# NilFoundation/vote-saver-protocol

Hardware: AMD Instinct MI355X
Metric: G1 MSM points/sec at 2^20 (Groth16 prover hot path) (higher is better)
Workload: dtype u32; 1 GPU; 2^20-point BLS12-381 G1 Pippenger MSM per GPU, PLAIN bases k_i*G (no table of window multiples; the library's 28-bit-limb copy keeps phi(P) = (beta x, y) beside every P for the endomorphism split), uniform scalars, bases and scalars resident in HBM; N ranks = one 2^20*N-point MSM sharded by contiguous chunk, RCCL all-gather of Jacobian partial sums + fold; points_per_gpu=1048576, window_bits=16, windows=8, endomorphism_split=True, msms_in_flight=4, bases_precomputed_window_multiples=False, bases_memory_bytes_per_point=352

## Files before the change

vote_saver_protocol_amd/csrc/fp28.h:

```cpp
#pragma once
#include "curve.h"

namespace vsp {

struct Fp28 {
    uint32_t l[14];
    VSP_HD static Fp28 zero() { Fp28 r; for (int i = 0; i < 14; i++) r.l[i] = 0; return r; }
};
VSP_HD bool is_zero(const Fp28 &a) { uint32_t o = 0; for (int i = 0; i < 14; i++) o |= a.l[i]; return o == 0; }
struct alignas(128) Affine28 { Fp28 x, y; };
static_assert(sizeof(Fp28) == 56 && sizeof(Affine28) == 128, "G1 table rows are one 128-byte line");
struct XYZZ28 { Fp28 X, Y, ZZ, ZZZ; };
struct Fp2x28 { Fp28 c0, c1; VSP_HD static Fp2x28 zero() { Fp2x28 r; r.c0 = Fp28::zero(); r.c1 = Fp28::zero(); return r; } };
struct Fp28L { Fp28 v; VSP_HD static Fp28L zero() { Fp28L r; r.v = Fp28::zero(); return r; } };
VSP_HD bool is_zero(const Fp2x28 &a) { return is_zero(a.c0) && is_zero(a.c1); }
struct alignas(256) Affine28x2 { Fp28 xc0, xc1, yc0, yc1; };
static_assert(sizeof(Affine28x2) == 256, "G2 table rows are two 128-byte lines");

#if defined(__HIP_DEVICE_COMPILE__)
__device__ __forceinline__ Fp28 fp28_zero() { Fp28 r; for (int i = 0; i < 14; i++) r.l[i] = 0; return r; }
__device__ __forceinline__ Fp28 fp28_const(const uint32_t (&c)[14]) { Fp28 r; for (int i = 0; i < 14; i++) r.l[i] = c[i]; return r; }
__device__ __forceinline__ bool fp28_all_zero(const Fp28 &a) { uint32_t o = 0; for (int i = 0; i < 14; i++) o |= a.l[i]; return o == 0; }
__device__ __forceinline__ bool fp28_equals(const Fp28 &a, const uint32_t (&c)[14]) { uint32_t o = 0; for (int i = 0; i < 14; i++) o |= a.l[i] ^ c[i]; return o == 0; }

#if defined(VSP_PORTABLE_MUL)
__device__ __noinline__ void mont28_portable(uint32_t *r, const uint32_t *a, const uint32_t *b, const uint32_t *c, const uint32_t *d) {
    uint32_t m[14];
    uint64_t acc = 0;
    for (int k = 0; k < 27; k++) {
        for (int i = (k > 13 ? k - 13 : 0); i <= (k < 13 ? k : 13); i++) {
            acc += (uint64_t)a[i] * b[k - i];
            if (c) acc += (uint64_t)c[i] * d[k - i];
        }
        if (k < 14) {
            for (int i = 0; i < k; i++) acc += (uint64_t)m[i] * FP28_P[k - i];
            m[k] = ((uint32_t)acc * 0xffcfffdu) & 0x0FFFFFFFu;
            acc += (uint64_t)m[k] * FP28_P[0];
        } else {
            for (int i = k - 13; i < 14; i++) acc += (uint64_t)m[i] * FP28_P[k - i];
            r[k - 14] = (uint32_t)acc & 0x0FFFFFFFu;
        }
        acc >>= 28;
    }
    r[13] = (uint32_t)acc;
}
__device__ __forceinline__ Fp28 mul28(const Fp28 &a, const Fp28 &b) { Fp28 r; mont28_portable(r.l, a.l, b.l, nullptr, nullptr); return r; }
__device__ __forceinline__ Fp28 sqr28(const Fp28 &a) { Fp28 r; mont28_portable(r.l, a.l, a.l, nullptr, nullptr); return r; }
__device__ __forceinline__ Fp28 mul28x2(const Fp28 &a, const Fp28 &b, const Fp28 &c, const Fp28 &d) { Fp28 r; mont28_portable(r.l, a.l, b.l, c.l, d.l); return r; }
#else
__device__ __forceinline__ Fp28 mul28(const Fp28 &a, const Fp28 &b) {
    Fp28 r;
    __builtin_amdgcn_sched_barrier(0);
    mont_mul28_asm(r.l, a.l, b.l);
    __builtin_amdgcn_sched_barrier(0);
    (void)&mont_mul28_holder<0>;
    return r;
}
__device__ __forceinline__ Fp28 sqr28(const Fp28 &a) {
    Fp28 r, a2;
#pragma unroll
    for (int i = 0; i < 14; i++) a2.l[i] = 2u * a.l[i];
    __builtin_amdgcn_sched_barrier(0);
    mont_sqr28_asm(r.l, a.l, a2.l);
    __builtin_amdgcn_sched_barrier(0);
    (void)&mont_sqr28_holder<0>;
    return r;
}
__device__ __forceinline__ Fp28 mul28x2(const Fp28 &a, const Fp28 &b, const Fp28 &c, const Fp28 &d) {
    Fp28 r;
    __builtin_amdgcn_sched_barrier(0);
    mont_mul28x2_asm(r.l, a.l, b.l, c.l, d.l);
    __builtin_amdgcn_sched_barrier(0);
    (void)&mont_mul28x2_holder<0>;
    return r;
}
#endif
__device__ __forceinline__ Fp28 sub28(const Fp28 &a, const uint32_t (&K)[14], const Fp28 &b) {
    Fp28 r;
#pragma unroll
    for (int i = 0; i < 14; i++) r.l[i] = a.l[i] + K[i] - b.l[i];
    return r;
}
__device__ __forceinline__ Fp28 neg28(const uint32_t (&K)[14], const Fp28 &b) {
    Fp28 r;
#pragma unroll
    for (int i = 0; i < 14; i++) r.l[i] = K[i] - b.l[i];
    return r;
}
__device__ __forceinline__ Fp28 norm28(const Fp28 &a) {
    Fp28 r;
    uint32_t c = 0;
#pragma unroll
    for (int i = 0; i < 13; i++) { uint32_t t = a.l[i] + c; r.l[i] = t & 0x0FFFFFFFu; c = t >> 28; }
    r.l[13] = a.l[13] + c;
    return r;
}
__device__ __forceinline__ bool fp28_product_is_zero(const Fp28 &a) { return fp28_all_zero(a) || fp28_equals(a, FP28_P); }

__device__ __forceinline__ Fp28 fp_to_fp28(const Fp &m) {
    __builtin_amdgcn_sched_barrier(0);
    Fp c = from_mont(m);
    __builtin_amdgcn_sched_barrier(0);
    Fp28 s;
#pragma unroll
    for (int i = 0; i < 14; i++) {
        const int bit = 28 * i, w = bit >> 5, sh = bit & 31;
        uint64_t v = c.l[w];
        if (w + 1 < 12) v |= (uint64_t)c.l[w + 1] << 32;
        s.l[i] = (uint32_t)(v >> sh) & (i < 13 ? 0x0FFFFFFFu : 0xFFFFFFFFu);
    }
    return mul28(s, fp28_const(FP28_R2));
}
__device__ __forceinline__ Fp fp28_to_fp(const Fp28 &x) {
    Fp28 one = fp28_zero(); one.l[0] = 1;
    Fp28 v = mul28(x, one);
    Fp28 d; uint32_t borrow = 0;
#pragma unroll
    for (int i = 0; i < 14; i++) {
        uint32_t t = v.l[i] - FP28_P[i] - borrow;
        borrow = (i < 13) ? ((t >> 28) & 1u) : (t >> 31);
        d.l[i] = (i < 13) ? (t & 0x0FFFFFFFu) : t;
    }
    if (!borrow) v = d;
    Fp c;
#pragma unroll
    for (int w = 0; w < 12; w++) {
        uint32_t acc = 0;
#pragma unroll
        for (int i = 0; i < 14; i++) {
            const int lo = 28 * i - 32 * w;
            if (lo > -28 && lo < 32) acc |= lo >= 0 ? (v.l[i] << lo) : (v.l[i] >> (-lo));
        }
        c.l[w] = acc;
    }
    __builtin_amdgcn_sched_barrier(0);
    Fp out = to_mont(c);
    __builtin_amdgcn_sched_barrier(0);
    return out;
}

__device__ __forceinline__ bool is_inf28(const Affine28 &p) { return fp28_all_zero(p.x) && fp28_all_zero(p.y); }
__device__ __forceinline__ bool is_inf28(const XYZZ28 &p) { return fp28_all_zero(p.ZZ); }
__device__ __forceinline__ XYZZ28 xyzz28_inf() { XYZZ28 r; r.X = r.Y = r.ZZ = r.ZZZ = fp28_zero(); return r; }
__device__ __forceinline__ XYZZ<Fp> xyzz28_to_fp(const XYZZ28 &a) {
    XYZZ<Fp> r;
    if (is_inf28(a)) return XYZZ<Fp>::inf();
    r.X = fp28_to_fp(a.X); r.Y = fp28_to_fp(a.Y); r.ZZ = fp28_to_fp(a.ZZ); r.ZZZ = fp28_to_fp(a.ZZZ);
    return r;
}

__device__ __forceinline__ bool madd28(XYZZ28 &acc, const Affine28 &q, bool negate) {
    if (is_inf28(q)) return true;
    Fp28 qy = negate ? neg28(FP28_K8_L1, q.y) : q.y;
    if (is_inf28(acc)) { acc.X = q.x; acc.Y = negate ? norm28(qy) : qy; acc.ZZ = fp28_const(FP28_ONE); acc.ZZZ = acc.ZZ; return true; }
    Fp28 U2 = mul28(q.x, acc.ZZ);
    Fp28 S2 = mul28(qy, acc.ZZZ);
    Fp28 P = norm28(sub28(U2, FP28_K32_L1, acc.X));
    Fp28 PP = sqr28(P);
    if (fp28_product_is_zero(PP)) return false;
    Fp28 R = norm28(sub28(S2, FP28_K32_L1, acc.Y));
    Fp28 PPP = mul28(P, PP);
    Fp28 Q = mul28(acc.X, PP);
    Fp28 s;
#pragma unroll
    for (int i = 0; i < 14; i++) s.l[i] = PPP.l[i] + 2u * Q.l[i];
    Fp28 X3 = norm28(sub28(sqr28(R), FP28_K8_L4, s));
    acc.Y = mul28x2(R, sub28(Q, FP28_K32_L1, X3), neg28(FP28_K32_L1, acc.Y), PPP);
    acc.X = X3;
    acc.ZZ = mul28(acc.ZZ, PP);
    acc.ZZZ = mul28(acc.ZZZ, PPP);
    return true;
}
__device__ __forceinline__ XYZZ<Fp28> xyzz28_from_fp(const XYZZ<Fp> &a) {
    XYZZ<Fp28> r;
    if (is_inf(a)) return XYZZ<Fp28>::inf();
    r.X = fp_to_fp28(a.X); r.Y = fp_to_fp28(a.Y); r.ZZ = fp_to_fp28(a.ZZ); r.ZZZ = fp_to_fp28(a.ZZZ);
    return r;
}
__device__ __forceinline__ XYZZ<Fp> xyzz28_to_fp(const XYZZ<Fp28> &a) {
    XYZZ<Fp> r;
    if (fp28_all_zero(a.ZZ)) return XYZZ<Fp>::inf();
    r.X = fp28_to_fp(a.X); r.Y = fp28_to_fp(a.Y); r.ZZ = fp28_to_fp(a.ZZ); r.ZZZ = fp28_to_fp(a.ZZZ);
    return r;
}
__device__ __forceinline__ XYZZ<Fp28> xyzz_dbl28(const XYZZ<Fp28> &a) {
    XYZZ<Fp28> r;
    Fp28 U;
#pragma unroll
    for (int i = 0; i < 14; i++) U.l[i] = 2u * a.Y.l[i];
    Fp28 V = mul28(U, U);
    Fp28 W = mul28(U, V);
    Fp28 S = mul28(a.X, V);
    Fp28 M = sqr28(a.X);
#pragma unroll
    for (int i = 0; i < 14; i++) M.l[i] *= 3u;
    M = norm28(M);
    Fp28 S2;
#pragma unroll
    for (int i = 0; i < 14; i++) S2.l[i] = 2u * S.l[i];
    r.X = norm28(sub28(sqr28(M), FP28_K8_L4, S2));
    r.Y = mul28x2(M, sub28(S, FP28_K32_L1, r.X), neg28(FP28_K32_L1, a.Y), W);
    r.ZZ = mul28(V, a.ZZ);
    r.ZZZ = mul28(W, a.ZZZ);
    return r;
}
__device__ __forceinline__ void xyzz_add(XYZZ<Fp28> &acc, const XYZZ<Fp28> &q) {
    if (fp28_all_zero(q.ZZ)) return;
    if (fp28_all_zero(acc.ZZ)) { acc = q; return; }
    Fp28 U1 = mul28(acc.X, q.ZZ), U2 = mul28(q.X, acc.ZZ);
    Fp28 S1 = mul28(acc.Y, q.ZZZ), S2 = mul28(q.Y, acc.ZZZ);
    Fp28 P = norm28(sub28(U2, FP28_K8_L1, U1));
    Fp28 PP = sqr28(P);
    Fp28 R = norm28(sub28(S2, FP28_K8_L1, S1));
    if (fp28_product_is_zero(PP)) {
        if (fp28_product_is_zero(sqr28(R))) acc = xyzz_dbl28(q); else acc = XYZZ<Fp28>::inf();
        return;
    }
    Fp28 PPP = mul28(P, PP);
    Fp28 Q = mul28(U1, PP);
    Fp28 s;
#pragma unroll
    for (int i = 0; i < 14; i++) s.l[i] = PPP.l[i] + 2u * Q.l[i];
    Fp28 X3 = norm28(sub28(sqr28(R), FP28_K8_L4, s));
    acc.Y = mul28x2(R, sub28(Q, FP28_K32_L1, X3), neg28(FP28_K8_L1, S1), PPP);
    acc.X = X3;
    acc.ZZ = mul28(mul28(acc.ZZ, q.ZZ), PP);
    acc.ZZZ = mul28(mul28(acc.ZZZ, q.ZZZ), PPP);
}


__device__ __forceinline__ Fp28 partner28(const Fp28 &a) {
    Fp28 r;
#pragma unroll
    for (int i = 0; i < 14; i++) r.l[i] = (uint32_t)__builtin_amdgcn_update_dpp(0, (int)a.l[i], 0xB1, 0xF, 0xF, false);
    return r;
}
__device__ __forceinline__ Fp28 select28(bool c, const Fp28 &a, const Fp28 &b) {
    Fp28 r;
#pragma unroll
    for (int i = 0; i < 14; i++) r.l[i] = c ? a.l[i] : b.l[i];
    return r;
}
__device__ __forceinline__ Fp28 mulF2(const Fp28 &a, const Fp28 &b, const uint32_t (&KB)[14]) {
    const bool hi = (threadIdx.x & 1) != 0;
    Fp28 ap = partner28(a), bp = partner28(b);
    Fp28 s1 = select28(hi, bp, b);
    Fp28 s2 = select28(hi, b, neg28(KB, bp));
    return mul28x2(a, s1, ap, s2);
}
__device__ __forceinline__ Fp28 sqrF2(const Fp28 &a, const uint32_t (&KA)[14]) {
    const bool hi = (threadIdx.x & 1) != 0;
    Fp28 ap = partner28(a), sum, dbl;
#pragma unroll
    for (int i = 0; i < 14; i++) { sum.l[i] = a.l[i] + ap.l[i]; dbl.l[i] = 2u * a.l[i]; }
    Fp28 x = select28(hi, ap, sum);
    Fp28 y = select28(hi, dbl, sub28(a, KA, ap));
    return mul28(x, y);
}
__device__ __forceinline__ bool fp28_small_is_zero(const Fp28 &a) {
    return fp28_all_zero(a) || fp28_equals(a, FP28_P) || fp28_equals(a, FP28_2P) || fp28_equals(a, FP28_3P);
}
__device__ __forceinline__ bool pair_all28(bool c) {
    int f = c ? 1 : 0;
    return (f & __builtin_amdgcn_update_dpp(0, f, 0xB1, 0xF, 0xF, false)) != 0;
}
struct AffineHalf28 { Fp28 x, y; };
struct XYZZHalf28 { Fp28 X, Y, ZZ, ZZZ; };
__device__ __forceinline__ XYZZHalf28 xyzz_half28_inf() { XYZZHalf28 r; r.X = r.Y = r.ZZ = r.ZZZ = fp28_zero(); return r; }

__device__ __forceinline__ bool madd28_g2(XYZZHalf28 &acc, const AffineHalf28 &q, bool negate) {
    const bool hi = (threadIdx.x & 1) != 0;
    if (pair_all28(fp28_all_zero(q.x) && fp28_all_zero(q.y))) return true;
    Fp28 qy = negate ? neg28(FP28_K8_L1, q.y) : q.y;
    if (pair_all28(fp28_all_zero(acc.ZZ))) {
        acc.X = q.x; acc.Y = qy;
        acc.ZZ = hi ? fp28_zero() : fp28_const(FP28_ONE); acc.ZZZ = acc.ZZ;
        return true;
    }
    Fp28 U2 = mulF2(q.x, acc.ZZ, FP28_K8_L1);
    Fp28 S2 = mulF2(qy, acc.ZZZ, FP28_K8_L1);
    Fp28 P = norm28(sub28(U2, FP28_K32_L1, acc.X));
    Fp28 PP = sqrF2(P, FP28_K64_L1);
    if (pair_all28(fp28_small_is_zero(PP))) return false;
    Fp28 R = norm28(sub28(S2, FP28_K32_L4, acc.Y));
    Fp28 PPP = mulF2(P, PP, FP28_K8_L1);
    Fp28 Q = mulF2(acc.X, PP, FP28_K8_L1);
    Fp28 s;
#pragma unroll
    for (int i = 0; i < 14; i++) s.l[i] = PPP.l[i] + 2u * Q.l[i];
    Fp28 X3 = norm28(sub28(sqrF2(R, FP28_K64_L1), FP28_K8_L4, s));
    Fp28 D = sub28(Q, FP28_K32_L1, X3);
    Fp28 t1 = mulF2(R, D, FP28_K64_L4);
    Fp28 t2 = mulF2(acc.Y, PPP, FP28_K8_L1);
    acc.Y = sub28(t1, FP28_K8_L1, t2);
    acc.X = X3;
    acc.ZZ = mulF2(acc.ZZ, PP, FP28_K8_L1);
    acc.ZZZ = mulF2(acc.ZZZ, PPP, FP28_K8_L1);
    return true;
}

__device__ __forceinline__ bool is_zero(const Fp28L &a) { return pair_all28(fp28_all_zero(a.v)); }
__device__ __forceinline__ XYZZ<Fp28L> xyzz_dbl28_g2(const XYZZ<Fp28L> &a) {
    XYZZ<Fp28L> r;
    Fp28 Yn = norm28(a.Y.v), U;
#pragma unroll
    for (int i = 0; i < 14; i++) U.l[i] = 2u * Yn.l[i];
    U = norm28(U);
    Fp28 V = sqrF2(U, FP28_K32_L1);
    Fp28 W = mulF2(U, V, FP28_K8_L1);
    Fp28 S = mulF2(a.X.v, V, FP28_K8_L1);
    Fp28 M = sqrF2(a.X.v, FP28_K32_L1);
#pragma unroll
    for (int i = 0; i < 14; i++) M.l[i] *= 3u;
    M = norm28(M);
    Fp28 S2;
#pragma unroll
    for (int i = 0; i < 14; i++) S2.l[i] = 2u * S.l[i];
    Fp28 X3 = norm28(sub28(sqrF2(M, FP28_K8_L1), FP28_K8_L4, S2));
    Fp28 D = sub28(S, FP28_K32_L1, X3);
    Fp28 t1 = mulF2(M, D, FP28_K64_L4);
    Fp28 t2 = mulF2(Yn, W, FP28_K8_L1);
    r.X.v = X3;
    r.Y.v = sub28(t1, FP28_K8_L1, t2);
    r.ZZ.v = mulF2(V, a.ZZ.v, FP28_K8_L1);
    r.ZZZ.v = mulF2(W, a.ZZZ.v, FP28_K8_L1);
    return r;
}
__device__ __forceinline__ void xyzz_add(XYZZ<Fp28L> &acc, const XYZZ<Fp28L> &q) {
    if (pair_all28(fp28_all_zero(q.ZZ.v))) return;
    if (pair_all28(fp28_all_zero(acc.ZZ.v))) { acc = q; return; }
    Fp28 U1 = mulF2(acc.X.v, q.ZZ.v, FP28_K8_L1), U2 = mulF2(q.X.v, acc.ZZ.v, FP28_K8_L1);
    Fp28 S1 = mulF2(acc.Y.v, q.ZZZ.v, FP28_K8_L1), S2 = mulF2(q.Y.v, acc.ZZZ.v, FP28_K8_L1);
    Fp28 P = norm28(sub28(U2, FP28_K8_L1, U1));
    Fp28 PP = sqrF2(P, FP28_K32_L1);
    Fp28 R = norm28(sub28(S2, FP28_K8_L1, S1));
    if (pair_all28(fp28_product_is_zero(PP))) {
        if (pair_all28(fp28_product_is_zero(sqrF2(R, FP28_K32_L1)))) acc = xyzz_dbl28_g2(q); else acc = XYZZ<Fp28L>::inf();
        return;
    }
    Fp28 PPP = mulF2(P, PP, FP28_K8_L1);
    Fp28 Q = mulF2(U1, PP, FP28_K8_L1);
    Fp28 s;
#pragma unroll
    for (int i = 0; i < 14; i++) s.l[i] = PPP.l[i] + 2u * Q.l[i];
    Fp28 X3 = norm28(sub28(sqrF2(R, FP28_K32_L1), FP28_K8_L4, s));
    Fp28 D = sub28(Q, FP28_K32_L1, X3);
    Fp28 t1 = mulF2(R, D, FP28_K64_L4);
    Fp28 t2 = mulF2(S1, PPP, FP28_K8_L1);
    acc.Y.v = sub28(t1, FP28_K8_L1, t2);
    acc.X.v = X3;
    acc.ZZ.v = mulF2(mulF2(acc.ZZ.v, q.ZZ.v, FP28_K8_L1), PP, FP28_K8_L1);
    acc.ZZZ.v = mulF2(mulF2(acc.ZZZ.v, q.ZZZ.v, FP28_K8_L1), PPP, FP28_K8_L1);
}
#else
__device__ __forceinline__ void xyzz_add(XYZZ<Fp28> &, const XYZZ<Fp28> &) {}
__device__ __forceinline__ void xyzz_add(XYZZ<Fp28L> &, const XYZZ<Fp28L> &) {}
#endif

}
```

vote_saver_protocol_amd/csrc/mont_asm_gfx950.h:

```cpp
#pragma once
#include <stdint.h>

namespace vsp {

template <class P> __device__ __attribute__((noinline, used)) void mont_mul_holder_12() {
    static_assert(P::N == 12, "limb count");
    asm volatile(
        "s_branch .Lvsp_mm_12_end\n\t"
        ".p2align 8\n\t"
        "vsp_mm_12:\n\t"
        "s_mov_b32 s0, %[p0]\n\t"
        "s_mov_b32 s1, %[p1]\n\t"
        "s_mov_b32 s2, %[p2]\n\t"
        "s_mov_b32 s3, %[p3]\n\t"
        "s_mov_b32 s4, %[p4]\n\t"
        "s_mov_b32 s5, %[p5]\n\t"
        "s_mov_b32 s6, %[p6]\n\t"
        "s_mov_b32 s7, %[p7]\n\t"
        "s_mov_b32 s8, %[p8]\n\t"
        "s_mov_b32 s9, %[p9]\n\t"
        "s_mov_b32 s10, %[p10]\n\t"
        "s_mov_b32 s11, %[p11]\n\t"
        "s_mov_b32 s12, %[inv]\n\t"
        "v_mov_b32 v36, 0\n\t"
// ... 955 lines not shown
        "v_addc_co_u32 v27, vcc, 0, v27, vcc\n\t"
        "v_mad_u64_u32 v[24:25], vcc, v22, s6, v[24:25]\n\t"
        "v_addc_co_u32 v27, vcc, 0, v27, vcc\n\t"
        "v_mad_u64_u32 v[24:25], vcc, v7, v13, v[24:25]\n\t"
        "v_addc_co_u32 v27, vcc, 0, v27, vcc\n\t"
        "v_mad_u64_u32 v[24:25], vcc, v23, s5, v[24:25]\n\t"
        "v_addc_co_u32 v27, vcc, 0, v27, vcc\n\t"
        "v_mov_b32 v20, v24\n\t"
        "v_mov_b32 v26, v25\n\t"
        "v_mad_u64_u32 v[26:27], vcc, v6, v15, v[26:27]\n\t"
        "v_addc_co_u32_e64 v25, vcc, 0, 0, vcc\n\t"
        "v_mad_u64_u32 v[26:27], vcc, v22, s7, v[26:27]\n\t"
        "v_addc_co_u32 v25, vcc, 0, v25, vcc\n\t"
        "v_mad_u64_u32 v[26:27], vcc, v7, v14, v[26:27]\n\t"
        "v_addc_co_u32 v25, vcc, 0, v25, vcc\n\t"
        "v_mad_u64_u32 v[26:27], vcc, v23, s6, v[26:27]\n\t"
        "v_addc_co_u32 v25, vcc, 0, v25, vcc\n\t"
        "v_mov_b32 v21, v26\n\t"
        "v_mov_b32 v24, v27\n\t"
        "v_mad_u64_u32 v[24:25], vcc, v7, v15, v[24:25]\n\t"
        "v_addc_co_u32_e64 v27, vcc, 0, 0, vcc\n\t"
        "v_mad_u64_u32 v[24:25], vcc, v23, s7, v[24:25]\n\t"
        "v_addc_co_u32 v27, vcc, 0, v27, vcc\n\t"
        "v_mov_b32 v22, v24\n\t"
        "v_mov_b32 v26, v25\n\t"
        "v_mov_b32 v23, v26\n\t"
        "v_subrev_co_u32 v0, vcc, s0, v16\n\t"
        "v_mov_b32 v9, s1\n\t"
        "v_subb_co_u32 v1, vcc, v17, v9, vcc\n\t"
        "v_mov_b32 v10, s2\n\t"
        "v_subb_co_u32 v2, vcc, v18, v10, vcc\n\t"
        "v_mov_b32 v11, s3\n\t"
        "v_subb_co_u32 v3, vcc, v19, v11, vcc\n\t"
        "v_mov_b32 v12, s4\n\t"
        "v_subb_co_u32 v4, vcc, v20, v12, vcc\n\t"
        "v_mov_b32 v13, s5\n\t"
        "v_subb_co_u32 v5, vcc, v21, v13, vcc\n\t"
        "v_mov_b32 v14, s6\n\t"
        "v_subb_co_u32 v6, vcc, v22, v14, vcc\n\t"
        "v_mov_b32 v15, s7\n\t"
        "v_subb_co_u32 v7, vcc, v23, v15, vcc\n\t"
        "v_cndmask_b32 v16, v0, v16, vcc\n\t"
        "v_cndmask_b32 v17, v1, v17, vcc\n\t"
        "v_cndmask_b32 v18, v2, v18, vcc\n\t"
        "v_cndmask_b32 v19, v3, v19, vcc\n\t"
        "v_cndmask_b32 v20, v4, v20, vcc\n\t"
        "v_cndmask_b32 v21, v5, v21, vcc\n\t"
        "v_cndmask_b32 v22, v6, v22, vcc\n\t"
        "v_cndmask_b32 v23, v7, v23, vcc\n\t"
        "s_nop 4\n\t"
        "s_setpc_b64 s[30:31]\n\t"
        ".Lvsp_mm_8_end:\n\t"
        :
        : [p0] "i"(P::MOD[0]), [p1] "i"(P::MOD[1]), [p2] "i"(P::MOD[2]), [p3] "i"(P::MOD[3]), [p4] "i"(P::MOD[4]), [p5] "i"(P::MOD[5]), [p6] "i"(P::MOD[6]), [p7] "i"(P::MOD[7]), [inv] "i"(P::INV)
        : "vcc", "scc", "s30", "s31", "s0", "s1", "s2", "s3", "s4", "s5", "s6", "s7", "s8", "s9", "s10", "s11", "s12", "v0", "v1", "v2", "v3", "v4", "v5", "v6", "v7", "v8", "v9", "v10", "v11", "v12", "v13", "v14", "v15", "v16", "v17", "v18", "v19", "v20", "v21", "v22", "v23", "v24", "v25", "v26", "v27");
}

template <class P> __device__ __forceinline__ void mont_mul_asm_8(uint32_t *r, uint32_t *a, uint32_t *b) {
    asm("s_getpc_b64 s[30:31]\n\t"
        "s_add_u32 s30, s30, vsp_mm_8@rel32@lo+4\n\t"
        "s_addc_u32 s31, s31, vsp_mm_8@rel32@hi+12\n\t"
        "s_swappc_b64 s[30:31], s[30:31]"
        : "={v16}"(r[0]), "={v17}"(r[1]), "={v18}"(r[2]), "={v19}"(r[3]), "={v20}"(r[4]), "={v21}"(r[5]), "={v22}"(r[6]), "={v23}"(r[7]), "+{v0}"(a[0]), "+{v1}"(a[1]), "+{v2}"(a[2]), "+{v3}"(a[3]), "+{v4}"(a[4]), "+{v5}"(a[5]), "+{v6}"(a[6]), "+{v7}"(a[7]), "+{v8}"(b[0]), "+{v9}"(b[1]), "+{v10}"(b[2]), "+{v11}"(b[3]), "+{v12}"(b[4]), "+{v13}"(b[5]), "+{v14}"(b[6]), "+{v15}"(b[7])
        :
        : "vcc", "scc", "s30", "s31", "s0", "s1", "s2", "s3", "s4", "s5", "s6", "s7", "s8", "s9", "s10", "s11", "s12", "v24", "v25", "v26", "v27");
}

static constexpr uint32_t FP28_P[14] = {0xfffaaabu, 0xfefffffu, 0x3ffffb9u, 0xfffeb15u, 0x6241eabu, 0xa0f6b0fu, 0xf6730d2u, 0xf38512bu, 0x4774b84u, 0x4bacd76u, 0xba7b643u, 0xe69a4b1u, 0x1ea397fu, 0x1a011u};
static constexpr uint32_t FP28_ONE[14] = {0x347fcb8u, 0xd800000u, 0x2b119u, 0xcde6d2u, 0xc7212e0u, 0x83a2090u, 0x37669fu, 0xda0f73eu, 0x9b09b42u, 0x1297bb0u, 0x515d98fu, 0x12ca7cu, 0x659fcfau, 0x577au};
static constexpr uint32_t FP28_R2[14] = {0x10370edu, 0x6d1c345u, 0xe243d62u, 0xec45c53u, 0x3b1d65au, 0x93317du, 0xb4f36a0u, 0x5d74088u, 0xc10ea72u, 0x865d118u, 0x7320a75u, 0xfd5cd50u, 0xcc8a759u, 0xc8d4u};
static constexpr uint32_t FP28_K8_L1[14] = {0x1ffd5558u, 0x1f7ffffeu, 0x1ffffdceu, 0x1fff58a8u, 0x1120f55eu, 0x107b587au, 0x1b398694u, 0x19c2895eu, 0x13ba5c26u, 0x15d66bb1u, 0x1d3db219u, 0x134d258cu, 0x1f51cbfeu, 0xd0087u};
static constexpr uint32_t FP28_K8_L4[14] = {0x4ffd5558u, 0x4f7ffffbu, 0x4ffffdcbu, 0x4fff58a5u, 0x4120f55bu, 0x407b5877u, 0x4b398691u, 0x49c2895bu, 0x43ba5c23u, 0x45d66baeu, 0x4d3db216u, 0x434d2589u, 0x4f51cbfbu, 0xd0084u};
static constexpr uint32_t FP28_K32_L1[14] = {0x1ff55560u, 0x1dfffffeu, 0x1ffff73eu, 0x1ffd62a6u, 0x1483d57eu, 0x11ed61ebu, 0x1ce61a53u, 0x170a257du, 0x1ee9709du, 0x1759aec7u, 0x14f6c868u, 0x1d349636u, 0x1d472ffbu, 0x340222u};
static constexpr uint32_t FP28_K32_L4[14] = {0x4ff55560u, 0x4dfffffbu, 0x4ffff73bu, 0x4ffd62a3u, 0x4483d57bu, 0x41ed61e8u, 0x4ce61a50u, 0x470a257au, 0x4ee9709au, 0x4759aec4u, 0x44f6c865u, 0x4d349633u, 0x4d472ff8u, 0x34021fu};
static constexpr uint32_t FP28_K64_L1[14] = {0x1feaaac0u, 0x1bfffffeu, 0x1fffee7eu, 0x1ffac54eu, 0x1907aafeu, 0x13dac3d7u, 0x19cc34a7u, 0x1e144afcu, 0x1dd2e13bu, 0x1eb35d90u, 0x19ed90d1u, 0x1a692c6du, 0x1a8e5ff8u, 0x680446u};
static constexpr uint32_t FP28_K64_L4[14] = {0x4feaaac0u, 0x4bfffffbu, 0x4fffee7bu, 0x4ffac54bu, 0x4907aafbu, 0x43dac3d4u, 0x49cc34a4u, 0x4e144af9u, 0x4dd2e138u, 0x4eb35d8du, 0x49ed90ceu, 0x4a692c6au, 0x4a8e5ff5u, 0x680443u};
static constexpr uint32_t FP28_2P[14] = {0xfff5556u, 0xfdfffffu, 0x7ffff73u, 0xfffd62au, 0xc483d57u, 0x41ed61eu, 0xece61a5u, 0xe70a257u, 0x8ee9709u, 0x9759aecu, 0x74f6c86u, 0xcd34963u, 0x3d472ffu, 0x34022u};
static constexpr uint32_t FP28_3P[14] = {0xfff0001u, 0xfcfffffu, 0xbffff2du, 0xfffc13fu, 0x26c5c03u, 0xe2e412eu, 0xe359277u, 0xda8f383u, 0xd65e28eu, 0xe306862u, 0x2f722c9u, 0xb3cee15u, 0x5beac7fu, 0x4e033u};
template <int Instance> __device__ __attribute__((noinline, used)) void mont_mul28_holder() {
    asm volatile(
        "s_branch .Lvsp_mm28_end\n\t"
        ".p2align 8\n\t"
        "vsp_mm28:\n\t"
        "s_mov_b32 s0, 0xfffaaab\n\t"
        "s_mov_b32 s1, 0xfefffff\n\t"
        "s_mov_b32 s2, 0x3ffffb9\n\t"
        "s_mov_b32 s3, 0xfffeb15\n\t"
        "s_mov_b32 s4, 0x6241eab\n\t"
        "s_mov_b32 s5, 0xa0f6b0f\n\t"
        "s_mov_b32 s6, 0xf6730d2\n\t"
        "s_mov_b32 s7, 0xf38512b\n\t"
        "s_mov_b32 s8, 0x4774b84\n\t"
        "s_mov_b32 s9, 0x4bacd76\n\t"
        "s_mov_b32 s10, 0xba7b643\n\t"
        "s_mov_b32 s11, 0xe69a4b1\n\t"
        "s_mov_b32 s12, 0x1ea397f\n\t"
        "s_mov_b32 s13, 0x1a011\n\t"
        "s_mov_b32 s14, 0xffcfffd\n\t"
        "s_mov_b32 s15, 0xfffffff\n\t"
        "v_mov_b32 v42, 0\n\t"
        "v_mov_b32 v43, 0\n\t"
        "v_mad_u64_u32 v[42:43], vcc, v0, v14, v[42:43]\n\t"
        "v_mul_lo_u32 v44, v42, s14\n\t"
        "v_and_b32 v28, s15, v44\n\t"
        "v_mad_u64_u32 v[42:43], vcc, v28, s0, v[42:43]\n\t"
        "v_lshrrev_b64 v[42:43], 28, v[42:43]\n\t"
        "v_mad_u64_u32 v[42:43], vcc, v0, v15, v[42:43]\n\t"
        "v_mad_u64_u32 v[42:43], vcc, v1, v14, v[42:43]\n\t"
        "v_mad_u64_u32 v[42:43], vcc, v28, s1, v[42:43]\n\t"
        "v_mul_lo_u32 v44, v42, s14\n\t"
        "v_and_b32 v29, s15, v44\n\t"
        "v_mad_u64_u32 v[42:43], vcc, v29, s0, v[42:43]\n\t"
        "v_lshrrev_b64 v[42:43], 28, v[42:43]\n\t"
        "v_mad_u64_u32 v[42:43], vcc, v0, v16, v[42:43]\n\t"
        "v_mad_u64_u32 v[42:43], vcc, v1, v15, v[42:43]\n\t"
        "v_mad_u64_u32 v[42:43], vcc, v2, v14, v[42:43]\n\t"
        "v_mad_u64_u32 v[42:43], vcc, v28, s2, v[42:43]\n\t"
        "v_mad_u64_u32 v[42:43], vcc, v29, s1, v[42:43]\n\t"
        "v_mul_lo_u32 v44, v42, s14\n\t"
        "v_and_b32 v30, s15, v44\n\t"
        "v_mad_u64_u32 v[42:43], vcc, v30, s0, v[42:43]\n\t"
        "v_lshrrev_b64 v[42:43], 28, v[42:43]\n\t"
        "v_mad_u64_u32 v[42:43], vcc, v0, v17, v[42:43]\n\t"
        "v_mad_u64_u32 v[42:43], vcc, v1, v16, v[42:43]\n\t"
        "v_mad_u64_u32 v[42:43], vcc, v2, v15, v[42:43]\n\t"
        "v_mad_u64_u32 v[42:43], vcc, v3, v14, v[42:43]\n\t"
        "v_mad_u64_u32 v[42:43], vcc, v28, s3, v[42:43]\n\t"
        "v_mad_u64_u32 v[42:43], vcc, v29, s2, v[42:43]\n\t"
        "v_mad_u64_u32 v[42:43], vcc, v30, s1, v[42:43]\n\t"
        "v_mul_lo_u32 v44, v42, s14\n\t"
        "v_and_b32 v31, s15, v44\n\t"
        "v_mad_u64_u32 v[42:43], vcc, v31, s0, v[42:43]\n\t"
        "v_lshrrev_b64 v[42:43], 28, v[42:43]\n\t"
        "v_mad_u64_u32 v[42:43], vcc, v0, v18, v[42:43]\n\t"
        "v_mad_u64_u32 v[42:43], vcc, v1, v17, v[42:43]\n\t"
        "v_mad_u64_u32 v[42:43], vcc, v2, v16, v[42:43]\n\t"
        "v_mad_u64_u32 v[42:43], vcc, v3, v15, v[42:43]\n\t"
        "v_mad_u64_u32 v[42:43], vcc, v4, v14, v[42:43]\n\t"
        "v_mad_u64_u32 v[42:43], vcc, v28, s4, v[42:43]\n\t"
        "v_mad_u64_u32 v[42:43], vcc, v29, s3, v[42:43]\n\t"
        "v_mad_u64_u32 v[42:43], vcc, v30, s2, v[42:43]\n\t"
        "v_mad_u64_u32 v[42:43], vcc, v31, s1, v[42:43]\n\t"
        "v_mul_lo_u32 v44, v42, s14\n\t"
        "v_and_b32 v32, s15, v44\n\t"
        "v_mad_u64_u32 v[42:43], vcc, v32, s0, v[42:43]\n\t"
        "v_lshrrev_b64 v[42:43], 28, v[42:43]\n\t"
        "v_mad_u64_u32 v[42:43], vcc, v0, v19, v[42:43]\n\t"
        "v_mad_u64_u32 v[42:43], vcc, v1, v18, v[42:43]\n\t"
        "v_mad_u64_u32 v[42:43], vcc, v2, v17, v[42:43]\n\t"
        "v_mad_u64_u32 v[42:43], vcc, v3, v16, v[42:43]\n\t"
        "v_mad_u64_u32 v[42:43], vcc, v4, v15, v[42:43]\n\t"
        "v_mad_u64_u32 v[42:43], vcc, v5, v14, v[42:43]\n\t"
        "v_mad_u64_u32 v[42:43], vcc, v28, s5, v[42:43]\n\t"
        "v_mad_u64_u32 v[42:43], vcc, v29, s4, v[42:43]\n\t"
        "v_mad_u64_u32 v[42:43], vcc, v30, s3, v[42:43]\n\t"
        "v_mad_u64_u32 v[42:43], vcc, v31, s2, v[42:43]\n\t"
        "v_mad_u64_u32 v[42:43], vcc, v32, s1, v[42:43]\n\t"
        "v_mul_lo_u32 v44, v42, s14\n\t"
        "v_and_b32 v33, s15, v44\n\t"
        "v_mad_u64_u32 v[42:43], vcc, v33, s0, v[42:43]\n\t"
        "v_lshrrev_b64 v[42:43], 28, v[42:43]\n\t"
        "v_mad_u64_u32 v[42:43], vcc, v0, v20, v[42:43]\n\t"
        "v_mad_u64_u32 v[42:43], vcc, v1, v19, v[42:43]\n\t"
        "v_mad_u64_u32 v[42:43], vcc, v2, v18, v[42:43]\n\t"
        "v_mad_u64_u32 v[42:43], vcc, v3, v17, v[42:43]\n\t"
        "v_mad_u64_u32 v[42:43], vcc, v4, v16, v[42:43]\n\t"
// ... 329 lines not shown
        "v_mad_u64_u32 v[42:43], vcc, v11, v23, v[42:43]\n\t"
        "v_mad_u64_u32 v[42:43], vcc, v12, v22, v[42:43]\n\t"
        "v_mad_u64_u32 v[42:43], vcc, v13, v21, v[42:43]\n\t"
        "v_mad_u64_u32 v[42:43], vcc, v35, s13, v[42:43]\n\t"
        "v_mad_u64_u32 v[42:43], vcc, v36, s12, v[42:43]\n\t"
        "v_mad_u64_u32 v[42:43], vcc, v37, s11, v[42:43]\n\t"
        "v_mad_u64_u32 v[42:43], vcc, v38, s10, v[42:43]\n\t"
        "v_mad_u64_u32 v[42:43], vcc, v39, s9, v[42:43]\n\t"
        "v_mad_u64_u32 v[42:43], vcc, v40, s8, v[42:43]\n\t"
        "v_mad_u64_u32 v[42:43], vcc, v41, s7, v[42:43]\n\t"
        "v_and_b32 v34, s15, v42\n\t"
        "v_lshrrev_b64 v[42:43], 28, v[42:43]\n\t"
        "v_mad_u64_u32 v[42:43], vcc, v8, v27, v[42:43]\n\t"
        "v_mad_u64_u32 v[42:43], vcc, v9, v26, v[42:43]\n\t"
        "v_mad_u64_u32 v[42:43], vcc, v10, v25, v[42:43]\n\t"
        "v_mad_u64_u32 v[42:43], vcc, v11, v24, v[42:43]\n\t"
        "v_mad_u64_u32 v[42:43], vcc, v12, v23, v[42:43]\n\t"
        "v_mad_u64_u32 v[42:43], vcc, v13, v22, v[42:43]\n\t"
        "v_mad_u64_u32 v[42:43], vcc, v36, s13, v[42:43]\n\t"
        "v_mad_u64_u32 v[42:43], vcc, v37, s12, v[42:43]\n\t"
        "v_mad_u64_u32 v[42:43], vcc, v38, s11, v[42:43]\n\t"
        "v_mad_u64_u32 v[42:43], vcc, v39, s10, v[42:43]\n\t"
        "v_mad_u64_u32 v[42:43], vcc, v40, s9, v[42:43]\n\t"
        "v_mad_u64_u32 v[42:43], vcc, v41, s8, v[42:43]\n\t"
        "v_and_b32 v35, s15, v42\n\t"
        "v_lshrrev_b64 v[42:43], 28, v[42:43]\n\t"
        "v_mad_u64_u32 v[42:43], vcc, v9, v27, v[42:43]\n\t"
        "v_mad_u64_u32 v[42:43], vcc, v10, v26, v[42:43]\n\t"
        "v_mad_u64_u32 v[42:43], vcc, v11, v25, v[42:43]\n\t"
        "v_mad_u64_u32 v[42:43], vcc, v12, v24, v[42:43]\n\t"
        "v_mad_u64_u32 v[42:43], vcc, v13, v23, v[42:43]\n\t"
        "v_mad_u64_u32 v[42:43], vcc, v37, s13, v[42:43]\n\t"
        "v_mad_u64_u32 v[42:43], vcc, v38, s12, v[42:43]\n\t"
        "v_mad_u64_u32 v[42:43], vcc, v39, s11, v[42:43]\n\t"
        "v_mad_u64_u32 v[42:43], vcc, v40, s10, v[42:43]\n\t"
        "v_mad_u64_u32 v[42:43], vcc, v41, s9, v[42:43]\n\t"
        "v_and_b32 v36, s15, v42\n\t"
        "v_lshrrev_b64 v[42:43], 28, v[42:43]\n\t"
        "v_mad_u64_u32 v[42:43], vcc, v10, v27, v[42:43]\n\t"
        "v_mad_u64_u32 v[42:43], vcc, v11, v26, v[42:43]\n\t"
        "v_mad_u64_u32 v[42:43], vcc, v12, v25, v[42:43]\n\t"
        "v_mad_u64_u32 v[42:43], vcc, v13, v24, v[42:43]\n\t"
        "v_mad_u64_u32 v[42:43], vcc, v38, s13, v[42:43]\n\t"
        "v_mad_u64_u32 v[42:43], vcc, v39, s12, v[42:43]\n\t"
        "v_mad_u64_u32 v[42:43], vcc, v40, s11, v[42:43]\n\t"
        "v_mad_u64_u32 v[42:43], vcc, v41, s10, v[42:43]\n\t"
        "v_and_b32 v37, s15, v42\n\t"
        "v_lshrrev_b64 v[42:43], 28, v[42:43]\n\t"
        "v_mad_u64_u32 v[42:43], vcc, v11, v27, v[42:43]\n\t"
        "v_mad_u64_u32 v[42:43], vcc, v12, v26, v[42:43]\n\t"
        "v_mad_u64_u32 v[42:43], vcc, v13, v25, v[42:43]\n\t"
        "v_mad_u64_u32 v[42:43], vcc, v39, s13, v[42:43]\n\t"
        "v_mad_u64_u32 v[42:43], vcc, v40, s12, v[42:43]\n\t"
        "v_mad_u64_u32 v[42:43], vcc, v41, s11, v[42:43]\n\t"
        "v_and_b32 v38, s15, v42\n\t"
        "v_lshrrev_b64 v[42:43], 28, v[42:43]\n\t"
        "v_mad_u64_u32 v[42:43], vcc, v12, v27, v[42:43]\n\t"
        "v_mad_u64_u32 v[42:43], vcc, v13, v26, v[42:43]\n\t"
        "v_mad_u64_u32 v[42:43], vcc, v40, s13, v[42:43]\n\t"
        "v_mad_u64_u32 v[42:43], vcc, v41, s12, v[42:43]\n\t"
        "v_and_b32 v39, s15, v42\n\t"
        "v_lshrrev_b64 v[42:43], 28, v[42:43]\n\t"
        "v_mad_u64_u32 v[42:43], vcc, v13, v27, v[42:43]\n\t"
        "v_mad_u64_u32 v[42:43], vcc, v41, s13, v[42:43]\n\t"
        "v_and_b32 v40, s15, v42\n\t"
        "v_lshrrev_b64 v[42:43], 28, v[42:43]\n\t"
        "v_mov_b32 v41, v42\n\t"
        "s_nop 4\n\t"
        "s_setpc_b64 s[30:31]\n\t"
        ".Lvsp_mm28_end:\n\t"
        :
        :
        : "vcc", "scc", "s30", "s31", "s0", "s1", "s2", "s3", "s4", "s5", "s6", "s7", "s8", "s9", "s10", "s11", "s12", "s13", "s14", "s15", "v0", "v1", "v2", "v3", "v4", "v5", "v6", "v7", "v8", "v9", "v10", "v11", "v12", "v13", "v14", "v15", "v16", "v17", "v18", "v19", "v20", "v21", "v22", "v23", "v24", "v25", "v26", "v27", "v28", "v29", "v30", "v31", "v32", "v33", "v34", "v35", "v36", "v37", "v38", "v39", "v40", "v41", "v42", "v43", "v44");
}
__device__ __forceinline__ void mont_mul28_asm(uint32_t *r, const uint32_t *a, const uint32_t *b) {
    asm("s_getpc_b64 s[30:31]\n\t"
        "s_add_u32 s30, s30, vsp_mm28@rel32@lo+4\n\t"
        "s_addc_u32 s31, s31, vsp_mm28@rel32@hi+12\n\t"
        "s_swappc_b64 s[30:31], s[30:31]"
        : "={v28}"(r[0]), "={v29}"(r[1]), "={v30}"(r[2]), "={v31}"(r[3]), "={v32}"(r[4]), "={v33}"(r[5]), "={v34}"(r[6]), "={v35}"(r[7]), "={v36}"(r[8]), "={v37}"(r[9]), "={v38}"(r[10]), "={v39}"(r[11]), "={v40}"(r[12]), "={v41}"(r[13])
        : "{v0}"(a[0]), "{v1}"(a[1]), "{v2}"(a[2]), "{v3}"(a[3]), "{v4}"(a[4]), "{v5}"(a[5]), "{v6}"(a[6]), "{v7}"(a[7]), "{v8}"(a[8]), "{v9}"(a[9]), "{v10}"(a[10]), "{v11}"(a[11]), "{v12}"(a[12]), "{v13}"(a[13]), "{v14}"(b[0]), "{v15}"(b[1]), "{v16}"(b[2]), "{v17}"(b[3]), "{v18}"(b[4]), "{v19}"(b[5]), "{v20}"(b[6]), "{v21}"(b[7]), "{v22}"(b[8]), "{v23}"(b[9]), "{v24}"(b[10]), "{v25}"(b[11]), "{v26}"(b[12]), "{v27}"(b[13])
        : "vcc", "scc", "s30", "s31", "s0", "s1", "s2", "s3", "s4", "s5", "s6", "s7", "s8", "s9", "s10", "s11", "s12", "s13", "s14", "s15", "v42", "v43", "v44");
}
template <int Instance> __device__ __attribute__((noinline, used)) void mont_sqr28_holder() {
    asm volatile(
        "s_branch .Lvsp_sq28_end\n\t"
        ".p2align 8\n\t"
        "vsp_sq28:\n\t"
        "s_mov_b32 s0, 0xfffaaab\n\t"
        "s_mov_b32 s1, 0xfefffff\n\t"
        "s_mov_b32 s2, 0x3ffffb9\n\t"
        "s_mov_b32 s3, 0xfffeb15\n\t"
        "s_mov_b32 s4, 0x6241eab\n\t"
        "s_mov_b32 s5, 0xa0f6b0f\n\t"
        "s_mov_b32 s6, 0xf6730d2\n\t"
        "s_mov_b32 s7, 0xf38512b\n\t"
        "s_mov_b32 s8, 0x4774b84\n\t"
        "s_mov_b32 s9, 0x4bacd76\n\t"
        "s_mov_b32 s10, 0xba7b643\n\t"
        "s_mov_b32 s11, 0xe69a4b1\n\t"
        "s_mov_b32 s12, 0x1ea397f\n\t"
        "s_mov_b32 s13, 0x1a011\n\t"
        "s_mov_b32 s14, 0xffcfffd\n\t"
        "s_mov_b32 s15, 0xfffffff\n\t"
        "v_mov_b32 v42, 0\n\t"
        "v_mov_b32 v43, 0\n\t"
        "v_mad_u64_u32 v[42:43], vcc, v0, v0, v[42:43]\n\t"
        "v_mul_lo_u32 v44, v42, s14\n\t"
        "v_and_b32 v28, s15, v44\n\t"
        "v_mad_u64_u32 v[42:43], vcc, v28, s0, v[42:43]\n\t"
        "v_lshrrev_b64 v[42:43], 28, v[42:43]\n\t"
        "v_mad_u64_u32 v[42:43], vcc, v0, v15, v[42:43]\n\t"
        "v_mad_u64_u32 v[42:43], vcc, v28, s1, v[42:43]\n\t"
        "v_mul_lo_u32 v44, v42, s14\n\t"
        "v_and_b32 v29, s15, v44\n\t"
        "v_mad_u64_u32 v[42:43], vcc, v29, s0, v[42:43]\n\t"
        "v_lshrrev_b64 v[42:43], 28, v[42:43]\n\t"
        "v_mad_u64_u32 v[42:43], vcc, v0, v16, v[42:43]\n\t"
        "v_mad_u64_u32 v[42:43], vcc, v1, v1, v[42:43]\n\t"
        "v_mad_u64_u32 v[42:43], vcc, v28, s2, v[42:43]\n\t"
        "v_mad_u64_u32 v[42:43], vcc, v29, s1, v[42:43]\n\t"
        "v_mul_lo_u32 v44, v42, s14\n\t"
        "v_and_b32 v30, s15, v44\n\t"
        "v_mad_u64_u32 v[42:43], vcc, v30, s0, v[42:43]\n\t"
        "v_lshrrev_b64 v[42:43], 28, v[42:43]\n\t"
        "v_mad_u64_u32 v[42:43], vcc, v0, v17, v[42:43]\n\t"
        "v_mad_u64_u32 v[42:43], vcc, v1, v16, v[42:43]\n\t"
        "v_mad_u64_u32 v[42:43], vcc, v28, s3, v[42:43]\n\t"
        "v_mad_u64_u32 v[42:43], vcc, v29, s2, v[42:43]\n\t"
        "v_mad_u64_u32 v[42:43], vcc, v30, s1, v[42:43]\n\t"
        "v_mul_lo_u32 v44, v42, s14\n\t"
        "v_and_b32 v31, s15, v44\n\t"
        "v_mad_u64_u32 v[42:43], vcc, v31, s0, v[42:43]\n\t"
        "v_lshrrev_b64 v[42:43], 28, v[42:43]\n\t"
        "v_mad_u64_u32 v[42:43], vcc, v0, v18, v[42:43]\n\t"
        "v_mad_u64_u32 v[42:43], vcc, v1, v17, v[42:43]\n\t"
        "v_mad_u64_u32 v[42:43], vcc, v2, v2, v[42:43]\n\t"
        "v_mad_u64_u32 v[42:43], vcc, v28, s4, v[42:43]\n\t"
        "v_mad_u64_u32 v[42:43], vcc, v29, s3, v[42:43]\n\t"
        "v_mad_u64_u32 v[42:43], vcc, v30, s2, v[42:43]\n\t"
        "v_mad_u64_u32 v[42:43], vcc, v31, s1, v[42:43]\n\t"
        "v_mul_lo_u32 v44, v42, s14\n\t"
        "v_and_b32 v32, s15, v44\n\t"
        "v_mad_u64_u32 v[42:43], vcc, v32, s0, v[42:43]\n\t"
        "v_lshrrev_b64 v[42:43], 28, v[42:43]\n\t"
        "v_mad_u64_u32 v[42:43], vcc, v0, v19, v[42:43]\n\t"
        "v_mad_u64_u32 v[42:43], vcc, v1, v18, v[42:43]\n\t"
        "v_mad_u64_u32 v[42:43], vcc, v2, v17, v[42:43]\n\t"
        "v_mad_u64_u32 v[42:43], vcc, v28, s5, v[42:43]\n\t"
        "v_mad_u64_u32 v[42:43], vcc, v29, s4, v[42:43]\n\t"
        "v_mad_u64_u32 v[42:43], vcc, v30, s3, v[42:43]\n\t"
        "v_mad_u64_u32 v[42:43], vcc, v31, s2, v[42:43]\n\t"
        "v_mad_u64_u32 v[42:43], vcc, v32, s1, v[42:43]\n\t"
        "v_mul_lo_u32 v44, v42, s14\n\t"
        "v_and_b32 v33, s15, v44\n\t"
        "v_mad_u64_u32 v[42:43], vcc, v33, s0, v[42:43]\n\t"
        "v_lshrrev_b64 v[42:43], 28, v[42:43]\n\t"
        "v_mad_u64_u32 v[42:43], vcc, v0, v20, v[42:43]\n\t"
        "v_mad_u64_u32 v[42:43], vcc, v1, v19, v[42:43]\n\t"
        "v_mad_u64_u32 v[42:43], vcc, v2, v18, v[42:43]\n\t"
        "v_mad_u64_u32 v[42:43], vcc, v3, v3, v[42:43]\n\t"
        "v_mad_u64_u32 v[42:43], vcc, v28, s6, v[42:43]\n\t"
        "v_mad_u64_u32 v[42:43], vcc, v29, s5, v[42:43]\n\t"
        "v_mad_u64_u32 v[42:43], vcc, v30, s4, v[42:43]\n\t"
        "v_mad_u64_u32 v[42:43], vcc, v31, s3, v[42:43]\n\t"
        "v_mad_u64_u32 v[42:43], vcc, v32, s2, v[42:43]\n\t"
        "v_mad_u64_u32 v[42:43], vcc, v33, s1, v[42:43]\n\t"
        "v_mul_lo_u32 v44, v42, s14\n\t"
        "v_and_b32 v34, s15, v44\n\t"
        "v_mad_u64_u32 v[42:43], vcc, v34, s0, v[42:43]\n\t"
        "v_lshrrev_b64 v[42:43], 28, v[42:43]\n\t"
// ... 238 lines not shown
        "v_mad_u64_u32 v[42:43], vcc, v36, s11, v[42:43]\n\t"
        "v_mad_u64_u32 v[42:43], vcc, v37, s10, v[42:43]\n\t"
        "v_mad_u64_u32 v[42:43], vcc, v38, s9, v[42:43]\n\t"
        "v_mad_u64_u32 v[42:43], vcc, v39, s8, v[42:43]\n\t"
        "v_mad_u64_u32 v[42:43], vcc, v40, s7, v[42:43]\n\t"
        "v_mad_u64_u32 v[42:43], vcc, v41, s6, v[42:43]\n\t"
        "v_and_b32 v33, s15, v42\n\t"
        "v_lshrrev_b64 v[42:43], 28, v[42:43]\n\t"
        "v_mad_u64_u32 v[42:43], vcc, v7, v27, v[42:43]\n\t"
        "v_mad_u64_u32 v[42:43], vcc, v8, v26, v[42:43]\n\t"
        "v_mad_u64_u32 v[42:43], vcc, v9, v25, v[42:43]\n\t"
        "v_mad_u64_u32 v[42:43], vcc, v10, v10, v[42:43]\n\t"
        "v_mad_u64_u32 v[42:43], vcc, v35, s13, v[42:43]\n\t"
        "v_mad_u64_u32 v[42:43], vcc, v36, s12, v[42:43]\n\t"
        "v_mad_u64_u32 v[42:43], vcc, v37, s11, v[42:43]\n\t"
        "v_mad_u64_u32 v[42:43], vcc, v38, s10, v[42:43]\n\t"
        "v_mad_u64_u32 v[42:43], vcc, v39, s9, v[42:43]\n\t"
        "v_mad_u64_u32 v[42:43], vcc, v40, s8, v[42:43]\n\t"
        "v_mad_u64_u32 v[42:43], vcc, v41, s7, v[42:43]\n\t"
        "v_and_b32 v34, s15, v42\n\t"
        "v_lshrrev_b64 v[42:43], 28, v[42:43]\n\t"
        "v_mad_u64_u32 v[42:43], vcc, v8, v27, v[42:43]\n\t"
        "v_mad_u64_u32 v[42:43], vcc, v9, v26, v[42:43]\n\t"
        "v_mad_u64_u32 v[42:43], vcc, v10, v25, v[42:43]\n\t"
        "v_mad_u64_u32 v[42:43], vcc, v36, s13, v[42:43]\n\t"
        "v_mad_u64_u32 v[42:43], vcc, v37, s12, v[42:43]\n\t"
        "v_mad_u64_u32 v[42:43], vcc, v38, s11, v[42:43]\n\t"
        "v_mad_u64_u32 v[42:43], vcc, v39, s10, v[42:43]\n\t"
        "v_mad_u64_u32 v[42:43], vcc, v40, s9, v[42:43]\n\t"
        "v_mad_u64_u32 v[42:43], vcc, v41, s8, v[42:43]\n\t"
        "v_and_b32 v35, s15, v42\n\t"
        "v_lshrrev_b64 v[42:43], 28, v[42:43]\n\t"
        "v_mad_u64_u32 v[42:43], vcc, v9, v27, v[42:43]\n\t"
        "v_mad_u64_u32 v[42:43], vcc, v10, v26, v[42:43]\n\t"
        "v_mad_u64_u32 v[42:43], vcc, v11, v11, v[42:43]\n\t"
        "v_mad_u64_u32 v[42:43], vcc, v37, s13, v[42:43]\n\t"
        "v_mad_u64_u32 v[42:43], vcc, v38, s12, v[42:43]\n\t"
        "v_mad_u64_u32 v[42:43], vcc, v39, s11, v[42:43]\n\t"
        "v_mad_u64_u32 v[42:43], vcc, v40, s10, v[42:43]\n\t"
        "v_mad_u64_u32 v[42:43], vcc, v41, s9, v[42:43]\n\t"
        "v_and_b32 v36, s15, v42\n\t"
        "v_lshrrev_b64 v[42:43], 28, v[42:43]\n\t"
        "v_mad_u64_u32 v[42:43], vcc, v10, v27, v[42:43]\n\t"
        "v_mad_u64_u32 v[42:43], vcc, v11, v26, v[42:43]\n\t"
        "v_mad_u64_u32 v[42:43], vcc, v38, s13, v[42:43]\n\t"
        "v_mad_u64_u32 v[42:43], vcc, v39, s12, v[42:43]\n\t"
        "v_mad_u64_u32 v[42:43], vcc, v40, s11, v[42:43]\n\t"
        "v_mad_u64_u32 v[42:43], vcc, v41, s10, v[42:43]\n\t"
        "v_and_b32 v37, s15, v42\n\t"
        "v_lshrrev_b64 v[42:43], 28, v[42:43]\n\t"
        "v_mad_u64_u32 v[42:43], vcc, v11, v27, v[42:43]\n\t"
        "v_mad_u64_u32 v[42:43], vcc, v12, v12, v[42:43]\n\t"
        "v_mad_u64_u32 v[42:43], vcc, v39, s13, v[42:43]\n\t"
        "v_mad_u64_u32 v[42:43], vcc, v40, s12, v[42:43]\n\t"
        "v_mad_u64_u32 v[42:43], vcc, v41, s11, v[42:43]\n\t"
        "v_and_b32 v38, s15, v42\n\t"
        "v_lshrrev_b64 v[42:43], 28, v[42:43]\n\t"
        "v_mad_u64_u32 v[42:43], vcc, v12, v27, v[42:43]\n\t"
        "v_mad_u64_u32 v[42:43], vcc, v40, s13, v[42:43]\n\t"
        "v_mad_u64_u32 v[42:43], vcc, v41, s12, v[42:43]\n\t"
        "v_and_b32 v39, s15, v42\n\t"
        "v_lshrrev_b64 v[42:43], 28, v[42:43]\n\t"
        "v_mad_u64_u32 v[42:43], vcc, v13, v13, v[42:43]\n\t"
        "v_mad_u64_u32 v[42:43], vcc, v41, s13, v[42:43]\n\t"
        "v_and_b32 v40, s15, v42\n\t"
        "v_lshrrev_b64 v[42:43], 28, v[42:43]\n\t"
        "v_mov_b32 v41, v42\n\t"
        "s_nop 4\n\t"
        "s_setpc_b64 s[30:31]\n\t"
        ".Lvsp_sq28_end:\n\t"
        :
        :
        : "vcc", "scc", "s30", "s31", "s0", "s1", "s2", "s3", "s4", "s5", "s6", "s7", "s8", "s9", "s10", "s11", "s12", "s13", "s14", "s15", "v0", "v1", "v2", "v3", "v4", "v5", "v6", "v7", "v8", "v9", "v10", "v11", "v12", "v13", "v14", "v15", "v16", "v17", "v18", "v19", "v20", "v21", "v22", "v23", "v24", "v25", "v26", "v27", "v28", "v29", "v30", "v31", "v32", "v33", "v34", "v35", "v36", "v37", "v38", "v39", "v40", "v41", "v42", "v43", "v44");
}
__device__ __forceinline__ void mont_sqr28_asm(uint32_t *r, const uint32_t *a, const uint32_t *a2) {
    asm("s_getpc_b64 s[30:31]\n\t"
        "s_add_u32 s30, s30, vsp_sq28@rel32@lo+4\n\t"
        "s_addc_u32 s31, s31, vsp_sq28@rel32@hi+12\n\t"
        "s_swappc_b64 s[30:31], s[30:31]"
        : "={v28}"(r[0]), "={v29}"(r[1]), "={v30}"(r[2]), "={v31}"(r[3]), "={v32}"(r[4]), "={v33}"(r[5]), "={v34}"(r[6]), "={v35}"(r[7]), "={v36}"(r[8]), "={v37}"(r[9]), "={v38}"(r[10]), "={v39}"(r[11]), "={v40}"(r[12]), "={v41}"(r[13])
        : "{v0}"(a[0]), "{v1}"(a[1]), "{v2}"(a[2]), "{v3}"(a[3]), "{v4}"(a[4]), "{v5}"(a[5]), "{v6}"(a[6]), "{v7}"(a[7]), "{v8}"(a[8]), "{v9}"(a[9]), "{v10}"(a[10]), "{v11}"(a[11]), "{v12}"(a[12]), "{v13}"(a[13]), "{v14}"(a2[0]), "{v15}"(a2[1]), "{v16}"(a2[2]), "{v17}"(a2[3]), "{v18}"(a2[4]), "{v19}"(a2[5]), "{v20}"(a2[6]), "{v21}"(a2[7]), "{v22}"(a2[8]), "{v23}"(a2[9]), "{v24}"(a2[10]), "{v25}"(a2[11]), "{v26}"(a2[12]), "{v27}"(a2[13])
        : "vcc", "scc", "s30", "s31", "s0", "s1", "s2", "s3", "s4", "s5", "s6", "s7", "s8", "s9", "s10", "s11", "s12", "s13", "s14", "s15", "v42", "v43", "v44");
}
template <int Instance> __device__ __attribute__((noinline, used)) void mont_mul28x2_holder() {
    asm volatile(
        "s_branch .Lvsp_mm28x2_end\n\t"
        ".p2align 8\n\t"
        "vsp_mm28x2:\n\t"
        "s_mov_b32 s0, 0xfffaaab\n\t"
        "s_mov_b32 s1, 0xfefffff\n\t"
        "s_mov_b32 s2, 0x3ffffb9\n\t"
        "s_mov_b32 s3, 0xfffeb15\n\t"
        "s_mov_b32 s4, 0x6241eab\n\t"
        "s_mov_b32 s5, 0xa0f6b0f\n\t"
        "s_mov_b32 s6, 0xf6730d2\n\t"
        "s_mov_b32 s7, 0xf38512b\n\t"
        "s_mov_b32 s8, 0x4774b84\n\t"
        "s_mov_b32 s9, 0x4bacd76\n\t"
        "s_mov_b32 s10, 0xba7b643\n\t"
        "s_mov_b32 s11, 0xe69a4b1\n\t"
        "s_mov_b32 s12, 0x1ea397f\n\t"
        "s_mov_b32 s13, 0x1a011\n\t"
        "s_mov_b32 s14, 0xffcfffd\n\t"
        "s_mov_b32 s15, 0xfffffff\n\t"
        "v_mov_b32 v70, 0\n\t"
        "v_mov_b32 v71, 0\n\t"
        "v_mad_u64_u32 v[70:71], vcc, v0, v14, v[70:71]\n\t"
        "v_mad_u64_u32 v[70:71], vcc, v28, v42, v[70:71]\n\t"
        "v_mul_lo_u32 v72, v70, s14\n\t"
        "v_and_b32 v56, s15, v72\n\t"
        "v_mad_u64_u32 v[70:71], vcc, v56, s0, v[70:71]\n\t"
        "v_lshrrev_b64 v[70:71], 28, v[70:71]\n\t"
        "v_mad_u64_u32 v[70:71], vcc, v0, v15, v[70:71]\n\t"
        "v_mad_u64_u32 v[70:71], vcc, v28, v43, v[70:71]\n\t"
        "v_mad_u64_u32 v[70:71], vcc, v1, v14, v[70:71]\n\t"
        "v_mad_u64_u32 v[70:71], vcc, v29, v42, v[70:71]\n\t"
        "v_mad_u64_u32 v[70:71], vcc, v56, s1, v[70:71]\n\t"
        "v_mul_lo_u32 v72, v70, s14\n\t"
        "v_and_b32 v57, s15, v72\n\t"
        "v_mad_u64_u32 v[70:71], vcc, v57, s0, v[70:71]\n\t"
        "v_lshrrev_b64 v[70:71], 28, v[70:71]\n\t"
        "v_mad_u64_u32 v[70:71], vcc, v0, v16, v[70:71]\n\t"
        "v_mad_u64_u32 v[70:71], vcc, v28, v44, v[70:71]\n\t"
        "v_mad_u64_u32 v[70:71], vcc, v1, v15, v[70:71]\n\t"
        "v_mad_u64_u32 v[70:71], vcc, v29, v43, v[70:71]\n\t"
        "v_mad_u64_u32 v[70:71], vcc, v2, v14, v[70:71]\n\t"
        "v_mad_u64_u32 v[70:71], vcc, v30, v42, v[70:71]\n\t"
        "v_mad_u64_u32 v[70:71], vcc, v56, s2, v[70:71]\n\t"
        "v_mad_u64_u32 v[70:71], vcc, v57, s1, v[70:71]\n\t"
        "v_mul_lo_u32 v72, v70, s14\n\t"
        "v_and_b32 v58, s15, v72\n\t"
        "v_mad_u64_u32 v[70:71], vcc, v58, s0, v[70:71]\n\t"
        "v_lshrrev_b64 v[70:71], 28, v[70:71]\n\t"
        "v_mad_u64_u32 v[70:71], vcc, v0, v17, v[70:71]\n\t"
        "v_mad_u64_u32 v[70:71], vcc, v28, v45, v[70:71]\n\t"
        "v_mad_u64_u32 v[70:71], vcc, v1, v16, v[70:71]\n\t"
        "v_mad_u64_u32 v[70:71], vcc, v29, v44, v[70:71]\n\t"
        "v_mad_u64_u32 v[70:71], vcc, v2, v15, v[70:71]\n\t"
        "v_mad_u64_u32 v[70:71], vcc, v30, v43, v[70:71]\n\t"
        "v_mad_u64_u32 v[70:71], vcc, v3, v14, v[70:71]\n\t"
        "v_mad_u64_u32 v[70:71], vcc, v31, v42, v[70:71]\n\t"
        "v_mad_u64_u32 v[70:71], vcc, v56, s3, v[70:71]\n\t"
        "v_mad_u64_u32 v[70:71], vcc, v57, s2, v[70:71]\n\t"
        "v_mad_u64_u32 v[70:71], vcc, v58, s1, v[70:71]\n\t"
        "v_mul_lo_u32 v72, v70, s14\n\t"
        "v_and_b32 v59, s15, v72\n\t"
        "v_mad_u64_u32 v[70:71], vcc, v59, s0, v[70:71]\n\t"
        "v_lshrrev_b64 v[70:71], 28, v[70:71]\n\t"
        "v_mad_u64_u32 v[70:71], vcc, v0, v18, v[70:71]\n\t"
        "v_mad_u64_u32 v[70:71], vcc, v28, v46, v[70:71]\n\t"
        "v_mad_u64_u32 v[70:71], vcc, v1, v17, v[70:71]\n\t"
        "v_mad_u64_u32 v[70:71], vcc, v29, v45, v[70:71]\n\t"
        "v_mad_u64_u32 v[70:71], vcc, v2, v16, v[70:71]\n\t"
        "v_mad_u64_u32 v[70:71], vcc, v30, v44, v[70:71]\n\t"
        "v_mad_u64_u32 v[70:71], vcc, v3, v15, v[70:71]\n\t"
        "v_mad_u64_u32 v[70:71], vcc, v31, v43, v[70:71]\n\t"
        "v_mad_u64_u32 v[70:71], vcc, v4, v14, v[70:71]\n\t"
        "v_mad_u64_u32 v[70:71], vcc, v32, v42, v[70:71]\n\t"
        "v_mad_u64_u32 v[70:71], vcc, v56, s4, v[70:71]\n\t"
        "v_mad_u64_u32 v[70:71], vcc, v57, s3, v[70:71]\n\t"
        "v_mad_u64_u32 v[70:71], vcc, v58, s2, v[70:71]\n\t"
        "v_mad_u64_u32 v[70:71], vcc, v59, s1, v[70:71]\n\t"
        "v_mul_lo_u32 v72, v70, s14\n\t"
        "v_and_b32 v60, s15, v72\n\t"
        "v_mad_u64_u32 v[70:71], vcc, v60, s0, v[70:71]\n\t"
        "v_lshrrev_b64 v[70:71], 28, v[70:71]\n\t"
        "v_mad_u64_u32 v[70:71], vcc, v0, v19, v[70:71]\n\t"
        "v_mad_u64_u32 v[70:71], vcc, v28, v47, v[70:71]\n\t"
        "v_mad_u64_u32 v[70:71], vcc, v1, v18, v[70:71]\n\t"
        "v_mad_u64_u32 v[70:71], vcc, v29, v46, v[70:71]\n\t"
        "v_mad_u64_u32 v[70:71], vcc, v2, v17, v[70:71]\n\t"
// ... 525 lines not shown
        "v_mad_u64_u32 v[70:71], vcc, v40, v51, v[70:71]\n\t"
        "v_mad_u64_u32 v[70:71], vcc, v13, v22, v[70:71]\n\t"
        "v_mad_u64_u32 v[70:71], vcc, v41, v50, v[70:71]\n\t"
        "v_mad_u64_u32 v[70:71], vcc, v64, s13, v[70:71]\n\t"
        "v_mad_u64_u32 v[70:71], vcc, v65, s12, v[70:71]\n\t"
        "v_mad_u64_u32 v[70:71], vcc, v66, s11, v[70:71]\n\t"
        "v_mad_u64_u32 v[70:71], vcc, v67, s10, v[70:71]\n\t"
        "v_mad_u64_u32 v[70:71], vcc, v68, s9, v[70:71]\n\t"
        "v_mad_u64_u32 v[70:71], vcc, v69, s8, v[70:71]\n\t"
        "v_and_b32 v63, s15, v70\n\t"
        "v_lshrrev_b64 v[70:71], 28, v[70:71]\n\t"
        "v_mad_u64_u32 v[70:71], vcc, v9, v27, v[70:71]\n\t"
        "v_mad_u64_u32 v[70:71], vcc, v37, v55, v[70:71]\n\t"
        "v_mad_u64_u32 v[70:71], vcc, v10, v26, v[70:71]\n\t"
        "v_mad_u64_u32 v[70:71], vcc, v38, v54, v[70:71]\n\t"
        "v_mad_u64_u32 v[70:71], vcc, v11, v25, v[70:71]\n\t"
        "v_mad_u64_u32 v[70:71], vcc, v39, v53, v[70:71]\n\t"
        "v_mad_u64_u32 v[70:71], vcc, v12, v24, v[70:71]\n\t"
        "v_mad_u64_u32 v[70:71], vcc, v40, v52, v[70:71]\n\t"
        "v_mad_u64_u32 v[70:71], vcc, v13, v23, v[70:71]\n\t"
        "v_mad_u64_u32 v[70:71], vcc, v41, v51, v[70:71]\n\t"
        "v_mad_u64_u32 v[70:71], vcc, v65, s13, v[70:71]\n\t"
        "v_mad_u64_u32 v[70:71], vcc, v66, s12, v[70:71]\n\t"
        "v_mad_u64_u32 v[70:71], vcc, v67, s11, v[70:71]\n\t"
        "v_mad_u64_u32 v[70:71], vcc, v68, s10, v[70:71]\n\t"
        "v_mad_u64_u32 v[70:71], vcc, v69, s9, v[70:71]\n\t"
        "v_and_b32 v64, s15, v70\n\t"
        "v_lshrrev_b64 v[70:71], 28, v[70:71]\n\t"
        "v_mad_u64_u32 v[70:71], vcc, v10, v27, v[70:71]\n\t"
        "v_mad_u64_u32 v[70:71], vcc, v38, v55, v[70:71]\n\t"
        "v_mad_u64_u32 v[70:71], vcc, v11, v26, v[70:71]\n\t"
        "v_mad_u64_u32 v[70:71], vcc, v39, v54, v[70:71]\n\t"
        "v_mad_u64_u32 v[70:71], vcc, v12, v25, v[70:71]\n\t"
        "v_mad_u64_u32 v[70:71], vcc, v40, v53, v[70:71]\n\t"
        "v_mad_u64_u32 v[70:71], vcc, v13, v24, v[70:71]\n\t"
        "v_mad_u64_u32 v[70:71], vcc, v41, v52, v[70:71]\n\t"
        "v_mad_u64_u32 v[70:71], vcc, v66, s13, v[70:71]\n\t"
        "v_mad_u64_u32 v[70:71], vcc, v67, s12, v[70:71]\n\t"
        "v_mad_u64_u32 v[70:71], vcc, v68, s11, v[70:71]\n\t"
        "v_mad_u64_u32 v[70:71], vcc, v69, s10, v[70:71]\n\t"
        "v_and_b32 v65, s15, v70\n\t"
        "v_lshrrev_b64 v[70:71], 28, v[70:71]\n\t"
        "v_mad_u64_u32 v[70:71], vcc, v11, v27, v[70:71]\n\t"
        "v_mad_u64_u32 v[70:71], vcc, v39, v55, v[70:71]\n\t"
        "v_mad_u64_u32 v[70:71], vcc, v12, v26, v[70:71]\n\t"
        "v_mad_u64_u32 v[70:71], vcc, v40, v54, v[70:71]\n\t"
        "v_mad_u64_u32 v[70:71], vcc, v13, v25, v[70:71]\n\t"
        "v_mad_u64_u32 v[70:71], vcc, v41, v53, v[70:71]\n\t"
        "v_mad_u64_u32 v[70:71], vcc, v67, s13, v[70:71]\n\t"
        "v_mad_u64_u32 v[70:71], vcc, v68, s12, v[70:71]\n\t"
        "v_mad_u64_u32 v[70:71], vcc, v69, s11, v[70:71]\n\t"
        "v_and_b32 v66, s15, v70\n\t"
        "v_lshrrev_b64 v[70:71], 28, v[70:71]\n\t"
        "v_mad_u64_u32 v[70:71], vcc, v12, v27, v[70:71]\n\t"
        "v_mad_u64_u32 v[70:71], vcc, v40, v55, v[70:71]\n\t"
        "v_mad_u64_u32 v[70:71], vcc, v13, v26, v[70:71]\n\t"
        "v_mad_u64_u32 v[70:71], vcc, v41, v54, v[70:71]\n\t"
        "v_mad_u64_u32 v[70:71], vcc, v68, s13, v[70:71]\n\t"
        "v_mad_u64_u32 v[70:71], vcc, v69, s12, v[70:71]\n\t"
        "v_and_b32 v67, s15, v70\n\t"
        "v_lshrrev_b64 v[70:71], 28, v[70:71]\n\t"
        "v_mad_u64_u32 v[70:71], vcc, v13, v27, v[70:71]\n\t"
        "v_mad_u64_u32 v[70:71], vcc, v41, v55, v[70:71]\n\t"
        "v_mad_u64_u32 v[70:71], vcc, v69, s13, v[70:71]\n\t"
        "v_and_b32 v68, s15, v70\n\t"
        "v_lshrrev_b64 v[70:71], 28, v[70:71]\n\t"
        "v_mov_b32 v69, v70\n\t"
        "s_nop 4\n\t"
        "s_setpc_b64 s[30:31]\n\t"
        ".Lvsp_mm28x2_end:\n\t"
        :
        :
        : "vcc", "scc", "s30", "s31", "s0", "s1", "s2", "s3", "s4", "s5", "s6", "s7", "s8", "s9", "s10", "s11", "s12", "s13", "s14", "s15", "v0", "v1", "v2", "v3", "v4", "v5", "v6", "v7", "v8", "v9", "v10", "v11", "v12", "v13", "v14", "v15", "v16", "v17", "v18", "v19", "v20", "v21", "v22", "v23", "v24", "v25", "v26", "v27", "v28", "v29", "v30", "v31", "v32", "v33", "v34", "v35", "v36", "v37", "v38", "v39", "v40", "v41", "v42", "v43", "v44", "v45", "v46", "v47", "v48", "v49", "v50", "v51", "v52", "v53", "v54", "v55", "v56", "v57", "v58", "v59", "v60", "v61", "v62", "v63", "v64", "v65", "v66", "v67", "v68", "v69", "v70", "v71", "v72");
}
__device__ __forceinline__ void mont_mul28x2_asm(uint32_t *r, const uint32_t *a, const uint32_t *b, const uint32_t *c, const uint32_t *d) {
    asm("s_getpc_b64 s[30:31]\n\t"
        "s_add_u32 s30, s30, vsp_mm28x2@rel32@lo+4\n\t"
        "s_addc_u32 s31, s31, vsp_mm28x2@rel32@hi+12\n\t"
        "s_swappc_b64 s[30:31], s[30:31]"
        : "={v56}"(r[0]), "={v57}"(r[1]), "={v58}"(r[2]), "={v59}"(r[3]), "={v60}"(r[4]), "={v61}"(r[5]), "={v62}"(r[6]), "={v63}"(r[7]), "={v64}"(r[8]), "={v65}"(r[9]), "={v66}"(r[10]), "={v67}"(r[11]), "={v68}"(r[12]), "={v69}"(r[13])
        : "{v0}"(a[0]), "{v1}"(a[1]), "{v2}"(a[2]), "{v3}"(a[3]), "{v4}"(a[4]), "{v5}"(a[5]), "{v6}"(a[6]), "{v7}"(a[7]), "{v8}"(a[8]), "{v9}"(a[9]), "{v10}"(a[10]), "{v11}"(a[11]), "{v12}"(a[12]), "{v13}"(a[13]), "{v14}"(b[0]), "{v15}"(b[1]), "{v16}"(b[2]), "{v17}"(b[3]), "{v18}"(b[4]), "{v19}"(b[5]), "{v20}"(b[6]), "{v21}"(b[7]), "{v22}"(b[8]), "{v23}"(b[9]), "{v24}"(b[10]), "{v25}"(b[11]), "{v26}"(b[12]), "{v27}"(b[13]), "{v28}"(c[0]), "{v29}"(c[1]), "{v30}"(c[2]), "{v31}"(c[3]), "{v32}"(c[4]), "{v33}"(c[5]), "{v34}"(c[6]), "{v35}"(c[7]), "{v36}"(c[8]), "{v37}"(c[9]), "{v38}"(c[10]), "{v39}"(c[11]), "{v40}"(c[12]), "{v41}"(c[13]), "{v42}"(d[0]), "{v43}"(d[1]), "{v44}"(d[2]), "{v45}"(d[3]), "{v46}"(d[4]), "{v47}"(d[5]), "{v48}"(d[6]), "{v49}"(d[7]), "{v50}"(d[8]), "{v51}"(d[9]), "{v52}"(d[10]), "{v53}"(d[11]), "{v54}"(d[12]), "{v55}"(d[13])
        : "vcc", "scc", "s30", "s31", "s0", "s1", "s2", "s3", "s4", "s5", "s6", "s7", "s8", "s9", "s10", "s11", "s12", "s13", "s14", "s15", "v70", "v71", "v72");
}

static constexpr uint32_t FR29_R[9] = {0x1u, 0x1ffffff8u, 0x1f96ffbfu, 0x1b4805ffu, 0x1d80553bu, 0xc0404d0u, 0x1520cce7u, 0xa6533afu, 0x73eda7u};
static constexpr uint32_t FR29_ONE[9] = {0x1fffffbau, 0x22fu, 0x1cb61180u, 0xa4e5c00u, 0xee8b1a2u, 0x16e6aedfu, 0x1907f8bbu, 0x853ddf7u, 0x4d043fu};
static constexpr uint32_t FR29_R2[9] = {0xa71b3c0u, 0x1d32207eu, 0x1663d999u, 0x1c5abc93u, 0x3b58c44u, 0xbe37438u, 0x829f771u, 0x1660139eu, 0x27fd91u};
static constexpr uint32_t FR29_K2_L1[9] = {0x20000002u, 0x3fffffefu, 0x3f2dff7eu, 0x36900bfeu, 0x3b00aa76u, 0x380809a0u, 0x2a4199cdu, 0x34ca675eu, 0xe7db4du};
static constexpr uint32_t FR29_K4_L1[9] = {0x20000004u, 0x3fffffdfu, 0x3e5bfefeu, 0x2d2017feu, 0x360154eeu, 0x30101342u, 0x3483339cu, 0x2994cebdu, 0x1cfb69cu};
template <int Instance> __device__ __attribute__((noinline, used)) void mont_mul29_holder() {
    asm volatile(
        "s_branch .Lvsp_mm29_end\n\t"
        ".p2align 8\n\t"
        "vsp_mm29:\n\t"
        "s_mov_b32 s0, 0x1\n\t"
        "s_mov_b32 s1, 0x1ffffff8\n\t"
        "s_mov_b32 s2, 0x1f96ffbf\n\t"
        "s_mov_b32 s3, 0x1b4805ff\n\t"
        "s_mov_b32 s4, 0x1d80553b\n\t"
        "s_mov_b32 s5, 0xc0404d0\n\t"
        "s_mov_b32 s6, 0x1520cce7\n\t"
        "s_mov_b32 s7, 0xa6533af\n\t"
        "s_mov_b32 s8, 0x73eda7\n\t"
        "s_mov_b32 s9, 0x1fffffff\n\t"
        "v_mov_b32 v94, 0\n\t"
        "v_mov_b32 v95, 0\n\t"
        "v_mad_u64_u32 v[94:95], vcc, v64, v74, v[94:95]\n\t"
        "v_sub_u32 v73, 0, v94\n\t"
        "v_and_b32 v84, s9, v73\n\t"
        "v_mad_u64_u32 v[94:95], vcc, v84, s0, v[94:95]\n\t"
        "v_lshrrev_b64 v[94:95], 29, v[94:95]\n\t"
        "v_mad_u64_u32 v[94:95], vcc, v64, v75, v[94:95]\n\t"
        "v_mad_u64_u32 v[94:95], vcc, v65, v74, v[94:95]\n\t"
        "v_mad_u64_u32 v[94:95], vcc, v84, s1, v[94:95]\n\t"
        "v_sub_u32 v73, 0, v94\n\t"
        "v_and_b32 v85, s9, v73\n\t"
        "v_mad_u64_u32 v[94:95], vcc, v85, s0, v[94:95]\n\t"
        "v_lshrrev_b64 v[94:95], 29, v[94:95]\n\t"
        "v_mad_u64_u32 v[94:95], vcc, v64, v76, v[94:95]\n\t"
        "v_mad_u64_u32 v[94:95], vcc, v65, v75, v[94:95]\n\t"
        "v_mad_u64_u32 v[94:95], vcc, v66, v74, v[94:95]\n\t"
        "v_mad_u64_u32 v[94:95], vcc, v84, s2, v[94:95]\n\t"
        "v_mad_u64_u32 v[94:95], vcc, v85, s1, v[94:95]\n\t"
        "v_sub_u32 v73, 0, v94\n\t"
        "v_and_b32 v86, s9, v73\n\t"
        "v_mad_u64_u32 v[94:95], vcc, v86, s0, v[94:95]\n\t"
        "v_lshrrev_b64 v[94:95], 29, v[94:95]\n\t"
        "v_mad_u64_u32 v[94:95], vcc, v64, v77, v[94:95]\n\t"
        "v_mad_u64_u32 v[94:95], vcc, v65, v76, v[94:95]\n\t"
        "v_mad_u64_u32 v[94:95], vcc, v66, v75, v[94:95]\n\t"
        "v_mad_u64_u32 v[94:95], vcc, v67, v74, v[94:95]\n\t"
        "v_mad_u64_u32 v[94:95], vcc, v84, s3, v[94:95]\n\t"
        "v_mad_u64_u32 v[94:95], vcc, v85, s2, v[94:95]\n\t"
        "v_mad_u64_u32 v[94:95], vcc, v86, s1, v[94:95]\n\t"
        "v_sub_u32 v73, 0, v94\n\t"
        "v_and_b32 v87, s9, v73\n\t"
        "v_mad_u64_u32 v[94:95], vcc, v87, s0, v[94:95]\n\t"
        "v_lshrrev_b64 v[94:95], 29, v[94:95]\n\t"
        "v_mad_u64_u32 v[94:95], vcc, v64, v78, v[94:95]\n\t"
        "v_mad_u64_u32 v[94:95], vcc, v65, v77, v[94:95]\n\t"
        "v_mad_u64_u32 v[94:95], vcc, v66, v76, v[94:95]\n\t"
        "v_mad_u64_u32 v[94:95], vcc, v67, v75, v[94:95]\n\t"
        "v_mad_u64_u32 v[94:95], vcc, v68, v74, v[94:95]\n\t"
        "v_mad_u64_u32 v[94:95], vcc, v84, s4, v[94:95]\n\t"
        "v_mad_u64_u32 v[94:95], vcc, v85, s3, v[94:95]\n\t"
        "v_mad_u64_u32 v[94:95], vcc, v86, s2, v[94:95]\n\t"
        "v_mad_u64_u32 v[94:95], vcc, v87, s1, v[94:95]\n\t"
        "v_sub_u32 v73, 0, v94\n\t"
        "v_and_b32 v88, s9, v73\n\t"
        "v_mad_u64_u32 v[94:95], vcc, v88, s0, v[94:95]\n\t"
        "v_lshrrev_b64 v[94:95], 29, v[94:95]\n\t"
        "v_mad_u64_u32 v[94:95], vcc, v64, v79, v[94:95]\n\t"
        "v_mad_u64_u32 v[94:95], vcc, v65, v78, v[94:95]\n\t"
        "v_mad_u64_u32 v[94:95], vcc, v66, v77, v[94:95]\n\t"
        "v_mad_u64_u32 v[94:95], vcc, v67, v76, v[94:95]\n\t"
        "v_mad_u64_u32 v[94:95], vcc, v68, v75, v[94:95]\n\t"
        "v_mad_u64_u32 v[94:95], vcc, v69, v74, v[94:95]\n\t"
        "v_mad_u64_u32 v[94:95], vcc, v84, s5, v[94:95]\n\t"
        "v_mad_u64_u32 v[94:95], vcc, v85, s4, v[94:95]\n\t"
        "v_mad_u64_u32 v[94:95], vcc, v86, s3, v[94:95]\n\t"
        "v_mad_u64_u32 v[94:95], vcc, v87, s2, v[94:95]\n\t"
        "v_mad_u64_u32 v[94:95], vcc, v88, s1, v[94:95]\n\t"
        "v_sub_u32 v73, 0, v94\n\t"
        "v_and_b32 v89, s9, v73\n\t"
        "v_mad_u64_u32 v[94:95], vcc, v89, s0, v[94:95]\n\t"
        "v_lshrrev_b64 v[94:95], 29, v[94:95]\n\t"
// ... 404 lines not shown
```

vote_saver_protocol_amd/csrc/msm_impl.inc:

```
#include "common.h"
#include "lane_view.h"
#include "fp28.h"
#if VSP_MSM_GROUP == 1
#include "accum28_asm_gfx950.h"
#endif


namespace vsp {
namespace {

#if VSP_MSM_GROUP == 1
static constexpr uint32_t GLV_BETA_MONT[12] = {0x8671f071u, 0xcd03c9e4u, 0x1fcda5d2u, 0x5dab2246u, 0xd3851b95u, 0x587042afu, 0x01bacb9eu, 0x8eb60ebeu, 0x83d050d2u, 0x03f97d6eu, 0x54638741u, 0x18f02065u};
#else
static constexpr uint32_t GLV_BETA_MONT[12] = {0x798a64e8u, 0x30f1361bu, 0x7ece5a2au, 0xf3b8ddabu, 0xc61577f7u, 0x16a8ca3au, 0x74fd029bu, 0xc26a2ff8u, 0x60701c6eu, 0x3636b766u, 0x241b6160u, 0x051ba4abu};
#endif
__device__ __forceinline__ Fp glv_beta() { Fp b; for (int i = 0; i < 12; i++) b.l[i] = GLV_BETA_MONT[i]; return b; }
__device__ __forceinline__ void glv_apply(Fp &x) { x = mul(x, glv_beta()); }
__device__ __forceinline__ void glv_apply(Fp2 &x) { Fp b = glv_beta(); x.c0 = mul(x.c0, b); x.c1 = mul(x.c1, b); }
__device__ __forceinline__ void glv_apply(Fp2L &x) { x.v = mul(x.v, glv_beta()); }

template <class F> struct AccumWaves { static constexpr unsigned W = 2; };
template <class F>
__device__ __forceinline__ XYZZ<typename LaneView<F>::E> accumulate_part(const Affine<F> *__restrict__ bases, const uint32_t *__restrict__ sorted, const uint32_t *__restrict__ off,
                                                const uint32_t *__restrict__ suboff, const uint32_t *__restrict__ part_bucket, uint32_t q,
                                                XYZZ<F> *buckets, XYZZ<F> *partials, bool glv = false) {
    using LV = LaneView<F>; using E = typename LV::E;
    auto load_entry = [&](uint32_t e) {
        const uint32_t idx = e & 0x7fffffffu;
        Affine<E> p = LV::load(&bases[glv ? (idx >> 1) : idx]);
        if (glv && (idx & 1u)) glv_apply(p.x);
        return p;
    };
    const uint32_t g = part_bucket[q];
    const uint32_t part = q - suboff[g];
    const uint32_t parts = suboff[g + 1] - suboff[g];
    const uint32_t b0 = off[g], b1 = off[g + 1];
    const uint32_t len = parts == 1 ? b1 - b0 : part_len(b1 - b0, parts);
    uint32_t start = b0 + part * len;
    if (start > b1) start = b1;
    uint32_t end = start + len < b1 ? start + len : b1;
    XYZZ<E> acc = XYZZ<E>::inf();
    if (start < end) {
        uint32_t e_cur = sorted[start];
        uint32_t e_nxt = start + 1 < end ? sorted[start + 1] : 0u;
        Affine<E> p_cur = load_entry(e_cur);
        for (uint32_t i = start; i < end; i++) {
            const bool more = i + 1 < end;
            Affine<E> p_nxt = p_cur;
            if (more) p_nxt = load_entry(e_nxt);
            const uint32_t e_nn = i + 2 < end ? sorted[i + 2] : 0u;
            xyzz_madd(acc, p_cur, (e_cur >> 31) != 0);
            p_cur = p_nxt; e_cur = e_nxt; e_nxt = e_nn;
        }
    }
    LV::store(parts == 1 ? &buckets[g] : &partials[q], acc);
    return acc;
}
template <class F>
__global__ __launch_bounds__(MSM_THREADS, AccumWaves<F>::W) void k_accum(const Affine<F> *__restrict__ bases, const uint32_t *__restrict__ sorted,
                                                       const uint32_t *__restrict__ off, const uint32_t *__restrict__ suboff,
                                                       const uint32_t *__restrict__ perm, const uint32_t *__restrict__ part_bucket,
                                                       size_t G, unsigned T, XYZZ<F> *buckets, XYZZ<F> *partials) {
    size_t t = gid<F>();
    if (t >= suboff[G]) return;
    accumulate_part<F>(bases, sorted, off, suboff, part_bucket, perm[t], buckets, partials);
}
#if VSP_MSM_GROUP == 1
using Bucket28 = XYZZ<Fp28>;
__device__ __forceinline__ void store_part28(Bucket28 *dst, const XYZZ<Fp> &a) {
#if defined(__HIP_DEVICE_COMPILE__)
    *dst = xyzz28_from_fp(a);
#endif
}
#else
using Bucket28 = XYZZ<Fp2x28>;
__device__ __forceinline__ void store_part28(Bucket28 *dst, const XYZZ<Fp2L> &a) {
#if defined(__HIP_DEVICE_COMPILE__)
    Fp28 *row = reinterpret_cast<Fp28 *>(dst);
    const unsigned comp = threadIdx.x & 1;
    const bool inf = is_inf(a);
    row[comp] = inf ? Fp28::zero() : fp_to_fp28(a.X.v); row[2 + comp] = inf ? Fp28::zero() : fp_to_fp28(a.Y.v);
    row[4 + comp] = inf ? Fp28::zero() : fp_to_fp28(a.ZZ.v); row[6 + comp] = inf ? Fp28::zero() : fp_to_fp28(a.ZZZ.v);
#endif
}
#endif
template <class F>
__global__ __launch_bounds__(MSM_THREADS, AccumWaves<F>::W) void k_accum_redo(const Affine<F> *__restrict__ bases, const uint32_t *__restrict__ sorted,
                                                            const uint32_t *__restrict__ off, const uint32_t *__restrict__ suboff,
                                                            const uint32_t *__restrict__ part_bucket, XYZZ<F> *buckets, XYZZ<F> *partials,
                                                            const uint32_t *redo_list, const uint32_t *redo_count, bool glv, Bucket28 *b28, Bucket28 *p28) {
    const uint32_t count = *redo_count;
    for (size_t t = gid<F>(); t < count; t += (size_t)gridDim.x * blockDim.x / LaneView<F>::LANES) {
        const uint32_t q = redo_list[t];
        auto acc = accumulate_part<F>(bases, sorted, off, suboff, part_bucket, q, buckets, partials, glv);
        if (b28) {
            const uint32_t g = part_bucket[q];
            store_part28(suboff[g + 1] - suboff[g] == 1 ? &b28[g] : &p28[q], acc);
        }
    }
}

#ifndef VSP_ACCUM28_WAVES
#define VSP_ACCUM28_WAVES 2
#endif
#if VSP_MSM_GROUP == 1
__global__ __launch_bounds__(MSM_THREADS, VSP_ACCUM28_WAVES) void k_accum28_cxx(const Affine28 *__restrict__ bases, const uint32_t *__restrict__ sorted,
                                                           const uint32_t *__restrict__ off, const uint32_t *__restrict__ suboff,
                                                           const uint32_t *__restrict__ perm, const uint32_t *__restrict__ part_bucket,
                                                           size_t G, unsigned T, XYZZ<Fp28> *buckets, XYZZ<Fp28> *partials,
                                                           uint32_t *redo_list, uint32_t *redo_count) {
#if defined(__HIP_DEVICE_COMPILE__)
    size_t t = (size_t)blockIdx.x * blockDim.x + threadIdx.x;
    uint32_t S = suboff[G];
    if (t >= S) return;
    const uint32_t q = perm[t];
    const uint32_t g = part_bucket[q];
    const uint32_t part = q - suboff[g];
    const uint32_t parts = suboff[g + 1] - suboff[g];
    const uint32_t b0 = off[g], b1 = off[g + 1];
    const uint32_t len = parts == 1 ? b1 - b0 : part_len(b1 - b0, parts);
    uint32_t start = b0 + part * len;
    if (start > b1) start = b1;
    uint32_t end = start + len < b1 ? start + len : b1;
    XYZZ28 acc = xyzz28_inf();
    if (start < end) {
        uint32_t e_cur = sorted[start];
        uint32_t e_nxt = start + 1 < end ? sorted[start + 1] : 0u;
        Affine28 p_cur = bases[e_cur & 0x7fffffffu];
        for (uint32_t i = start; i < end; i++) {
            const bool more = i + 1 < end;
            Affine28 p_nxt = p_cur;
            if (more) p_nxt = bases[e_nxt & 0x7fffffffu];
            const uint32_t e_nn = i + 2 < end ? sorted[i + 2] : 0u;
            if (!madd28(acc, p_cur, (e_cur >> 31) != 0)) {
                redo_list[atomicAdd(redo_count, 1u)] = q;
                return;
            }
            p_cur = p_nxt; e_cur = e_nxt; e_nxt = e_nn;
        }
    }
    XYZZ<Fp28> out; out.X = acc.X; out.Y = acc.Y; out.ZZ = acc.ZZ; out.ZZZ = acc.ZZZ;
    if (parts == 1) buckets[g] = out; else partials[q] = out;
#endif
}
#ifdef VSP_DIAG_CLOCK
__device__ unsigned long long vsp_diag_clock_sums[4];
#endif
__global__ __launch_bounds__(MSM_THREADS, 3) void k_accum28(const Affine28 *__restrict__ bases, const uint32_t *__restrict__ sorted,
                                                           const uint32_t *__restrict__ off, const uint32_t *__restrict__ suboff,
                                                           const uint32_t *__restrict__ perm, const uint32_t *__restrict__ part_bucket,
                                                           size_t G, unsigned T, XYZZ<Fp28> *buckets, XYZZ<Fp28> *partials,
                                                           uint32_t *redo_list, uint32_t *redo_count) {
#if defined(__HIP_DEVICE_COMPILE__)
    const size_t t = (size_t)blockIdx.x * blockDim.x + threadIdx.x;
    const uint32_t S = suboff[G];
    if (t >= S) return;
    const uint32_t q = perm[t];
    const uint32_t g = part_bucket[q];
    const uint32_t part = q - suboff[g];
    const uint32_t parts = suboff[g + 1] - suboff[g];
    const uint32_t b0 = off[g], b1 = off[g + 1];
    const uint32_t len = parts == 1 ? b1 - b0 : part_len(b1 - b0, parts);
    uint32_t start = b0 + part * len;
    if (start > b1) start = b1;
    const uint32_t end = start + len < b1 ? start + len : b1;
    XYZZ<Fp28> out;
    uint32_t flag;
#ifdef VSP_DIAG_CLOCK
    unsigned long long dc_t0, dc_r0, dc_t1, dc_r1;
    asm volatile("s_memtime %0\n\ts_memrealtime %1\n\ts_waitcnt lgkmcnt(0)" : "=s"(dc_t0), "=s"(dc_r0) :: "memory");
#endif
    accum28_asm(out.X.l, flag, bases, sorted, start, end);
#ifdef VSP_DIAG_CLOCK
    asm volatile("s_memtime %0\n\ts_memrealtime %1\n\ts_waitcnt lgkmcnt(0)" : "=s"(dc_t1), "=s"(dc_r1) :: "memory");
// ... 8 lines not shown
__global__ __launch_bounds__(256) void k_table28(const Affine<Fp> *in, size_t n, Affine28 *out, bool glv) {
#if defined(__HIP_DEVICE_COMPILE__)
    size_t i = (size_t)blockIdx.x * blockDim.x + threadIdx.x;
    if (i >= n) return;
    Affine<Fp> p = in[i];
    Affine28 r;
    r.x = fp_to_fp28(p.x); r.y = fp_to_fp28(p.y);
    out[glv ? 2 * i : i] = r;
    if (glv) { glv_apply(p.x); r.x = fp_to_fp28(p.x); out[2 * i + 1] = r; }
#endif
}
#endif

#if VSP_MSM_GROUP == 2
__global__ __launch_bounds__(MSM_THREADS, VSP_ACCUM28_WAVES) void k_accum28(const Affine28x2 *__restrict__ bases, const uint32_t *__restrict__ sorted,
                                                           const uint32_t *__restrict__ off, const uint32_t *__restrict__ suboff,
                                                           const uint32_t *__restrict__ perm, const uint32_t *__restrict__ part_bucket,
                                                           size_t G, unsigned T, XYZZ<Fp2x28> *buckets, XYZZ<Fp2x28> *partials,
                                                           uint32_t *redo_list, uint32_t *redo_count) {
#if defined(__HIP_DEVICE_COMPILE__)
    const size_t t = ((size_t)blockIdx.x * blockDim.x + threadIdx.x) >> 1;
    const unsigned comp = threadIdx.x & 1;
    uint32_t S = suboff[G];
    if (t >= S) return;
    const uint32_t q = perm[t];
    const uint32_t g = part_bucket[q];
    const uint32_t part = q - suboff[g];
    const uint32_t parts = suboff[g + 1] - suboff[g];
    const uint32_t b0 = off[g], b1 = off[g + 1];
    const uint32_t len = parts == 1 ? b1 - b0 : part_len(b1 - b0, parts);
    uint32_t start = b0 + part * len;
    if (start > b1) start = b1;
    uint32_t end = start + len < b1 ? start + len : b1;
    auto load = [&](uint32_t e) {
        const Fp28 *row = reinterpret_cast<const Fp28 *>(&bases[e & 0x7fffffffu]);
        AffineHalf28 p; p.x = row[comp]; p.y = row[2 + comp]; return p;
    };
    XYZZHalf28 acc = xyzz_half28_inf();
    if (start < end) {
        uint32_t e_cur = sorted[start];
        uint32_t e_nxt = start + 1 < end ? sorted[start + 1] : 0u;
        AffineHalf28 p_cur = load(e_cur);
        for (uint32_t i = start; i < end; i++) {
            const bool more = i + 1 < end;
            AffineHalf28 p_nxt = p_cur;
            if (more) p_nxt = load(e_nxt);
            const uint32_t e_nn = i + 2 < end ? sorted[i + 2] : 0u;
            if (!madd28_g2(acc, p_cur, (e_cur >> 31) != 0)) {
                if (comp == 0) redo_list[atomicAdd(redo_count, 1u)] = q;
                return;
            }
            p_cur = p_nxt; e_cur = e_nxt; e_nxt = e_nn;
        }
    }
    Fp28 *dst = reinterpret_cast<Fp28 *>(parts == 1 ? &buckets[g] : &partials[q]);
    dst[comp] = acc.X; dst[2 + comp] = acc.Y; dst[4 + comp] = acc.ZZ; dst[6 + comp] = acc.ZZZ;
#endif
}
__global__ __launch_bounds__(256) void k_table28(const Affine<Fp2> *in, size_t n, Affine28x2 *out, bool glv) {
#if defined(__HIP_DEVICE_COMPILE__)
    size_t i = (size_t)blockIdx.x * blockDim.x + threadIdx.x;
    if (i >= n) return;
    Affine<Fp2> p = in[i];
    Affine28x2 r;
    r.xc0 = fp_to_fp28(p.x.c0); r.xc1 = fp_to_fp28(p.x.c1); r.yc0 = fp_to_fp28(p.y.c0); r.yc1 = fp_to_fp28(p.y.c1);
    out[glv ? 2 * i : i] = r;
    if (glv) { glv_apply(p.x); r.xc0 = fp_to_fp28(p.x.c0); r.xc1 = fp_to_fp28(p.x.c1); out[2 * i + 1] = r; }
#endif
}
#endif

template <class F, unsigned NT>
__device__ __forceinline__ XYZZ<typename LaneView<F>::E> block_sum(XYZZ<typename LaneView<F>::E> acc, XYZZ<typename LaneView<F>::E> *sh) {
    unsigned t = threadIdx.x;
    sh[t] = acc;
    __syncthreads();
    for (unsigned s = NT / 2; s >= LaneView<F>::LANES; s >>= 1) {
        if (t < s) { xyzz_add(acc, sh[t + s]); sh[t] = acc; }
        __syncthreads();
    }
    return acc;
}

template <class F> struct MsmBlock { static constexpr unsigned NT = 256; static constexpr unsigned NTL = NT / LaneView<F>::LANES; };
#ifndef VSP_MERGE_NT
#define VSP_MERGE_NT 256
#endif
template <class F> struct MergeBlock { static constexpr unsigned NT = VSP_MERGE_NT; static constexpr unsigned NTL = NT / LaneView<F>::LANES; };

static constexpr unsigned MERGE1_BLOCKS = 1024;
template <class F>
__device__ __forceinline__ void merge1_block(unsigned b, const uint32_t *heavy, const uint32_t *counters, const uint32_t *suboff,
                                             XYZZ<F> *partials, XYZZ<typename LaneView<F>::E> *sh) {
    using LV = LaneView<F>; using E = typename LV::E;
    constexpr unsigned NT = MergeBlock<F>::NT, NTL = MergeBlock<F>::NTL;
    const uint32_t nh = counters[0], maxparts = counters[4];
    if (!nh || maxparts <= NTL) return;
    const uint64_t items = (uint64_t)nh * ((maxparts + NTL - 1) / NTL);
    for (uint64_t i = b; i < items; i += MERGE1_BLOCKS) {
        const uint32_t h = (uint32_t)(i % nh), k = (uint32_t)(i / nh);
        const uint32_t g = heavy[h];
        const uint32_t q0 = suboff[g], q1 = suboff[g + 1];
        if (q1 - q0 <= NTL) continue;
        const uint64_t c0 = (uint64_t)q0 + (uint64_t)k * NTL;
        if (c0 >= q1) continue;
        const uint32_t q = (uint32_t)c0 + lid<F>();
        XYZZ<E> acc = q < q1 ? LV::load(&partials[q]) : XYZZ<E>::inf();
        acc = block_sum<F, NT>(acc, sh);
        if (lid<F>() == 0) LV::store(&partials[c0], acc);
        __syncthreads();
    }
}
template <class F>
__global__ __launch_bounds__(MergeBlock<F>::NT, 2) void k_merge2(const uint32_t *heavy, const uint32_t *counters, const uint32_t *suboff,
                                                             const XYZZ<F> *partials, XYZZ<F> *buckets) {
    using LV = LaneView<F>; using E = typename LV::E;
    constexpr unsigned NT = MergeBlock<F>::NT, NTL = MergeBlock<F>::NTL;
    __shared__ XYZZ<E> sh[NT];
    uint32_t nh = counters[0];
    for (uint32_t h = blockIdx.x; h < nh; h += gridDim.x) {
        uint32_t g = heavy[h];
        uint32_t q0 = suboff[g], q1 = suboff[g + 1];
        const uint32_t stride = (q1 - q0 <= NTL) ? 1u : NTL;
        XYZZ<E> acc = XYZZ<E>::inf();
        for (uint32_t q = q0 + lid<F>() * stride; q < q1; q += NTL * stride) xyzz_add(acc, LV::load(&partials[q]));
        acc = block_sum<F, NT>(acc, sh);
        if (lid<F>() == 0) LV::store(&buckets[g], acc);
        __syncthreads();
    }
}

template <class F, unsigned LPB>
__global__ __launch_bounds__(MergeBlock<F>::NT, 2) void k_merge_a(const uint32_t *medium, const uint32_t *heavy, const uint32_t *counters, const uint32_t *suboff,
                                                                XYZZ<F> *partials, XYZZ<F> *buckets, unsigned small_blocks) {
    using LV = LaneView<F>; using E = typename LV::E;
    constexpr unsigned NT = MergeBlock<F>::NT, NTL = MergeBlock<F>::NTL, PER_BLOCK = NTL / LPB;
    __shared__ XYZZ<E> sh[NT];
    if (blockIdx.x >= small_blocks) {
        const unsigned b = blockIdx.x - small_blocks;
        merge1_block<F>(b, heavy, counters, suboff, partials, sh);
        return;
    }
    const uint32_t nm = counters[2];
    const unsigned lt = lid<F>(), lane = lt % LPB, slot = lt / LPB;
    for (size_t base = (size_t)blockIdx.x * PER_BLOCK; base < nm; base += (size_t)small_blocks * PER_BLOCK) {
        const size_t t = base + slot;
        const bool live = t < nm;
        const uint32_t g = live ? medium[t] : 0u;
        const uint32_t q0 = live ? suboff[g] : 0u, q1 = live ? suboff[g + 1] : 0u;
        XYZZ<E> acc = XYZZ<E>::inf();
        for (uint32_t q = q0 + lane; q < q1; q += LPB) xyzz_add(acc, LV::load(&partials[q]));
        if constexpr (LPB > 1) {
            sh[threadIdx.x] = acc;
            __syncthreads();
            for (unsigned s = LPB / 2; s >= 1; s >>= 1) {
                if (lane < s) { xyzz_add(acc, sh[threadIdx.x + s * LV::LANES]); sh[threadIdx.x] = acc; }
                __syncthreads();
            }
        }
        if (live && lane == 0) LV::store(&buckets[g], acc);
    }
}

template <class F>
__global__ __launch_bounds__(MSM_THREADS, AccumWaves<F>::W) void k_shift_window(const Affine<F> *in, size_t n, unsigned c, XYZZ<F> *out) {
    using LV = LaneView<F>; using E = typename LV::E;
    size_t i = gid<F>();
    if (i >= n) return;
    XYZZ<E> acc = xyzz_from_affine(LV::load(&in[i]));
    for (unsigned k = 0; k < c; k++) acc = xyzz_dbl(acc);
    LV::store(&out[i], acc);
}
static constexpr unsigned PRE_CHUNK = 32;
template <class F>
__global__ __launch_bounds__(64) void k_batch_affine_mont(const XYZZ<F> *in, size_t n, F *pre, Affine<F> *out) {
    size_t t = (size_t)blockIdx.x * blockDim.x + threadIdx.x;
    size_t b = t * PRE_CHUNK, e = b + PRE_CHUNK < n ? b + PRE_CHUNK : n;
    if (b >= n) return;
    F acc = F::one();
    for (size_t i = b; i < e; i++) {
        pre[i] = acc;
        F z = in[i].ZZZ;
        if (!is_zero(z)) acc = mul(acc, z);
    }
    F ai = inv(acc);
    for (size_t i = e; i-- > b;) {
        XYZZ<F> p = in[i];
        Affine<F> r;
        if (is_zero(p.ZZ)) { r.x = F::zero(); r.y = F::zero(); }
        else {
            F zi3 = mul(ai, pre[i]);
            ai = mul(ai, p.ZZZ);
            F zi = mul(zi3, p.ZZ);
            F zi2 = sqr(zi);
            r.x = mul(p.X, zi2);
            r.y = mul(p.Y, zi3);
        }
        out[i] = r;
    }
}

__host__ __device__ __forceinline__ unsigned dims_n2(const MsmGeom &g) { return g.q2 ? (1u << g.q2) : 0u; }
__host__ __device__ __forceinline__ unsigned dims_per_w(const MsmGeom &g) { return (1u << g.q0) + (1u << g.q1) + dims_n2(g); }
template <class F> static void split_digits(MsmGeom &g, bool dimbits) {
    const unsigned qb = g.c - 1;
    unsigned maxq = 0; while ((2u << maxq) <= MsmBlock<F>::NTL) maxq++;
    if (qb <= 2 * maxq || (dimbits && qb <= 24)) { g.q0 = (qb + 1) / 2; g.q1 = qb - g.q0; g.q2 = 0; }
    else { g.q0 = qb / 3; g.q1 = (qb - g.q0) / 2; g.q2 = qb - g.q0 - g.q1; }
    g.bd = (g.q2 == 0 && g.q0 > 8) ? 12u : 8u;
}

template <class F> struct DimSumWaves { static constexpr unsigned MAX = 1024; };
template <> struct DimSumWaves<Fp28> { static constexpr unsigned MAX = 2048; };
template <> struct DimSumWaves<Fp2x28> { static constexpr unsigned MAX = 2048; };
template <class F, unsigned LPS>
__global__ __launch_bounds__(64, AccumWaves<F>::W) void k_dimsum(const XYZZ<F> *buckets, MsmGeom g, XYZZ<F> *dims) {
    using LV = LaneView<F>; using E = typename LV::E;
    constexpr unsigned LANES = LV::LANES, SPW = 64 / LANES / LPS;
    __shared__ XYZZ<E> sh[64];
    const unsigned n0 = 1u << g.q0, n1 = 1u << g.q1;
    const unsigned per_w = dims_per_w(g);
    const unsigned lt = threadIdx.x / LANES;
    const unsigned lane = lt % LPS;
    const unsigned sum_id = blockIdx.x * SPW + lt / LPS;
    const bool live = sum_id < g.Wr * per_w;
    const unsigned w = live ? sum_id / per_w : 0;
    const unsigned slot = live ? sum_id % per_w : 0;
    unsigned d, v;
    if (slot < n0) { d = 0; v = slot; } else if (slot < n0 + n1) { d = 1; v = slot - n0; } else { d = 2; v = slot - n0 - n1; }
    const unsigned qd = d == 0 ? g.q0 : (d == 1 ? g.q1 : g.q2);
    const unsigned items = live ? g.B >> qd : 0;
    const XYZZ<F> *bw = buckets + (size_t)w * g.B;
    XYZZ<E> acc = XYZZ<E>::inf();
    for (unsigned i = lane; i < items; i += LPS) {
        unsigned idx;
        if (d == 0) idx = (i << g.q0) | v;
        else if (d == 1) idx = ((i >> g.q0) << (g.q1 + g.q0)) | (v << g.q0) | (i & (n0 - 1));
        else idx = (v << (g.q1 + g.q0)) | i;
        xyzz_add(acc, LV::load(&bw[idx]));
    }
    sh[threadIdx.x] = acc;
    __syncthreads();
    for (unsigned s = LPS / 2; s >= 1; s >>= 1) {
        if (lane < s) { xyzz_add(acc, sh[threadIdx.x + s * LANES]); sh[threadIdx.x] = acc; }
        __syncthreads();
    }
    if (live && lane == 0) LV::store(&dims[(size_t)w * per_w + slot], acc);
}

struct DimSumPlan { unsigned lps[3]; unsigned wave0[4]; };
template <class F, bool PREFETCH>
__global__ __launch_bounds__(64, AccumWaves<F>::W) void k_dimsum_mixed(const XYZZ<F> *buckets, MsmGeom g, XYZZ<F> *dims, DimSumPlan pl) {
    using LV = LaneView<F>; using E = typename LV::E;
    constexpr unsigned LANES = LV::LANES, LL = 64 / LANES;
    __shared__ XYZZ<E> sh[64];
    const unsigned n0 = 1u << g.q0, n1 = 1u << g.q1, n2 = dims_n2(g);
    const unsigned per_w = dims_per_w(g);
    const unsigned d = blockIdx.x < pl.wave0[1] ? 0u : (blockIdx.x < pl.wave0[2] ? 1u : 2u);
    const unsigned LPS = pl.lps[d], SPW = LL / LPS;
    const unsigned nd = d == 0 ? n0 : (d == 1 ? n1 : n2), base = d == 0 ? 0u : (d == 1 ? n0 : n0 + n1);
    const unsigned lt = threadIdx.x / LANES;
    const unsigned lane = lt % LPS;
    const unsigned id = (blockIdx.x - pl.wave0[d]) * SPW + lt / LPS;
    const bool live = id < g.Wr * nd;
    const unsigned w = live ? id / nd : 0, v = live ? id % nd : 0;
    const unsigned qd = d == 0 ? g.q0 : (d == 1 ? g.q1 : g.q2);
    const unsigned items = live ? g.B >> qd : 0;
    const XYZZ<F> *bw = buckets + (size_t)w * g.B;
    auto index_of = [&](unsigned i) {
        if (d == 0) return (i << g.q0) | v;
        if (d == 1) return ((i >> g.q0) << (g.q1 + g.q0)) | (v << g.q0) | (i & (n0 - 1));
        return (v << (g.q1 + g.q0)) | i;
    };
    XYZZ<E> acc = XYZZ<E>::inf();
    if constexpr (LANES == 1 && PREFETCH) {
        XYZZ<E> nxt = lane < items ? LV::load(&bw[index_of(lane)]) : XYZZ<E>::inf();
        for (unsigned i = lane; i < items; i += LPS) {
            const XYZZ<E> cur = nxt;
            if (i + LPS < items) nxt = LV::load(&bw[index_of(i + LPS)]);
            xyzz_add(acc, cur);
        }
    } else {
        for (unsigned i = lane; i < items; i += LPS) xyzz_add(acc, LV::load(&bw[index_of(i)]));
    }
    sh[threadIdx.x] = acc;
    __syncthreads();
    for (unsigned s = LPS / 2; s >= 1; s >>= 1) {
        if (lane < s) { xyzz_add(acc, sh[threadIdx.x + s * LANES]); sh[threadIdx.x] = acc; }
        __syncthreads();
    }
    if (live && lane == 0) LV::store(&dims[(size_t)w * per_w + base + v], acc);
}
struct DimSumDensePlan { unsigned lps[3]; unsigned blk0[4]; };
static constexpr unsigned DIMSUM_DENSE_NT = 256;
template <class F>
__global__ __launch_bounds__(DIMSUM_DENSE_NT, AccumWaves<F>::W) void k_dimsum_dense(const XYZZ<F> *buckets, MsmGeom g, XYZZ<F> *dims, DimSumDensePlan pl) {
    using LV = LaneView<F>; using E = typename LV::E;
    static_assert(LV::LANES == 1, "the lane-pair form keeps k_dimsum_mixed");
    constexpr unsigned NT = DIMSUM_DENSE_NT;
    __shared__ XYZZ<E> sh[NT];
    const unsigned n0 = 1u << g.q0, n1 = 1u << g.q1, n2 = dims_n2(g);
    const unsigned per_w = dims_per_w(g);
    const unsigned d = blockIdx.x < pl.blk0[1] ? 0u : (blockIdx.x < pl.blk0[2] ? 1u : 2u);
    const unsigned LPS = pl.lps[d], SPB = NT / LPS;
    const unsigned nd = d == 0 ? n0 : (d == 1 ? n1 : n2), base = d == 0 ? 0u : (d == 1 ? n0 : n0 + n1);
    const unsigned qd = d == 0 ? g.q0 : (d == 1 ? g.q1 : g.q2);
    const unsigned id0 = (blockIdx.x - pl.blk0[d]) * SPB;
    const unsigned lane = threadIdx.x % LPS;
    {
        const unsigned id = id0 + threadIdx.x / LPS;
        const bool live = id < g.Wr * nd;
        const unsigned w = live ? id / nd : 0, v = live ? id % nd : 0;
        const unsigned items = live ? g.B >> qd : 0;
        const XYZZ<F> *bw = buckets + (size_t)w * g.B;
        auto index_of = [&](unsigned i) {
            if (d == 0) return (i << g.q0) | v;
            if (d == 1) return ((i >> g.q0) << (g.q1 + g.q0)) | (v << g.q0) | (i & (n0 - 1));
            return (v << (g.q1 + g.q0)) | i;
        };
        XYZZ<E> acc = XYZZ<E>::inf();
        for (unsigned i = lane; i < items; i += LPS) xyzz_add(acc, LV::load(&bw[index_of(i)]));
        sh[threadIdx.x] = acc;
    }
    __syncthreads();
    const unsigned wave_first = threadIdx.x & ~63u;
    for (unsigned s = LPS / 2; s >= 1; s >>= 1) {
        const unsigned A = SPB * s;
        if (wave_first < A) {
            const unsigned j = threadIdx.x;
            if (j < A) {
                const unsigned slot = (j / s) * LPS + j % s;
                XYZZ<E> acc = sh[slot];
                xyzz_add(acc, sh[slot + s]);
                if (s > 1) sh[slot] = acc;
                else {
                    const unsigned id = id0 + j;
                    if (id < g.Wr * nd) LV::store(&dims[(size_t)(id / nd) * per_w + base + id % nd], acc);
                }
            }
        }
        __syncthreads();
    }
}
template <class F> static DimSumPlan dimsum_plan(const MsmGeom &g, unsigned MAXW = 1024) {
    constexpr unsigned LL = 64 / LaneView<F>::LANES;
    const unsigned nd[3] = {1u << g.q0, 1u << g.q1, dims_n2(g)};
    const unsigned qd[3] = {g.q0, g.q1, g.q2};
    DimSumPlan pl;
    auto lg2 = [](unsigned x) { unsigned l = 0; while ((1u << l) < x) l++; return l; };
    auto waves_of = [&](unsigned d, unsigned lps) { return nd[d] ? (unsigned)(((size_t)g.Wr * nd[d] * lps + LL - 1) / LL) : 0u; };
    auto steps_of = [&](unsigned d, unsigned lps) { const unsigned items = g.B >> qd[d]; return nd[d] ? (items + lps - 1) / lps + lg2(lps) : 0u; };
    for (unsigned d = 0; d < 3; d++) {
        unsigned l = (g.B >> qd[d]) / 8; if (l < 8) l = 8; if (l > LL) l = LL;
        unsigned p = 8; while (p * 2 <= l) p *= 2;
        pl.lps[d] = nd[d] ? p : 8;
    }
    auto total = [&]() { return waves_of(0, pl.lps[0]) + waves_of(1, pl.lps[1]) + waves_of(2, pl.lps[2]); };
    if (total() > MAXW) { pl.wave0[3] = 0; return pl; }
    for (int guard = 0; guard < 16; guard++) {
        int pick = -1;
        for (unsigned d = 0; d < 3; d++) {
            if (!nd[d] || pl.lps[d] >= LL || steps_of(d, pl.lps[d] * 2) >= steps_of(d, pl.lps[d])) continue;
            if (total() - waves_of(d, pl.lps[d]) + waves_of(d, pl.lps[d] * 2) > MAXW) continue;
            if (pick < 0 || steps_of(d, pl.lps[d]) > steps_of((unsigned)pick, pl.lps[pick])) pick = (int)d;
        }
        if (pick < 0) break;
        pl.lps[pick] *= 2;
    }
    pl.wave0[0] = 0;
    for (unsigned d = 0; d < 3; d++) pl.wave0[d + 1] = pl.wave0[d] + waves_of(d, pl.lps[d]);
    return pl;
}

template <class F> struct WinOut { using type = F; };
template <> struct WinOut<Fp28> { using type = Fp; };
template <> struct WinOut<Fp2x28> { using type = Fp2; };
template <class F> __device__ __forceinline__ void store_win(XYZZ<F> *p, const XYZZ<typename LaneView<F>::E> &v) { LaneView<F>::store(p, v); }
__device__ __forceinline__ void store_win(XYZZ<Fp> *p, const XYZZ<Fp28> &v) {
#if defined(__HIP_DEVICE_COMPILE__)
    *p = xyzz28_to_fp(v);
#endif
}
__device__ __forceinline__ void store_win(XYZZ<Fp2> *p, const XYZZ<Fp28L> &v) {
#if defined(__HIP_DEVICE_COMPILE__)
    Fp *row = reinterpret_cast<Fp *>(p);
    const unsigned comp = threadIdx.x & 1;
    const bool inf = pair_all28(fp28_all_zero(v.ZZ.v));
    row[comp] = inf ? Fp::zero() : fp28_to_fp(v.X.v); row[2 + comp] = inf ? Fp::zero() : fp28_to_fp(v.Y.v);
    row[4 + comp] = inf ? Fp::zero() : fp28_to_fp(v.ZZ.v); row[6 + comp] = inf ? Fp::zero() : fp28_to_fp(v.ZZZ.v);
#endif
}
template <class F>
__global__ __launch_bounds__(MsmBlock<F>::NT, 2) void k_dimweight(const XYZZ<F> *dims, MsmGeom g, XYZZ<typename WinOut<F>::type> *winres) {
    using LV = LaneView<F>; using E = typename LV::E;
    constexpr unsigned NT = MsmBlock<F>::NT, NTL = MsmBlock<F>::NTL;
    __shared__ XYZZ<E> sh[NT];
    const unsigned n0 = 1u << g.q0, n1 = 1u << g.q1, n2 = dims_n2(g);
    const unsigned per_w = dims_per_w(g);
    const unsigned w = blockIdx.x / 3u, d = blockIdx.x % 3u;
    if (d == 2 && !g.q2) {
        if (lid<F>() == 0) store_win(&winres[(size_t)w * 4 + 2], XYZZ<E>::inf());
        return;
    }
    const unsigned cntv = d == 0 ? n0 : (d == 1 ? n1 : n2);
    const unsigned doff = d == 0 ? 0 : (d == 1 ? n0 : n0 + n1);
    const unsigned t = lid<F>();
    XYZZ<E> x = t < cntv ? LV::load(&dims[(size_t)w * per_w + doff + t]) : XYZZ<E>::inf();
    sh[at<F>(t)] = x;
    __syncthreads();
    for (unsigned s = 1; s < cntv; s <<= 1) {
        XYZZ<E> y = (t + s < NTL) ? sh[at<F>(t + s)] : XYZZ<E>::inf();
        __syncthreads();
        xyzz_add(x, y);
        sh[at<F>(t)] = x;
        __syncthreads();
    }
    XYZZ<E> tot = sh[at<F>(0)];
    __syncthreads();
    XYZZ<E> acc = (t >= 1 && t < cntv) ? x : XYZZ<E>::inf();
    acc = block_sum<F, NT>(acc, sh);
    if (t == 0) {
        store_win(&winres[(size_t)w * 4 + d], acc);
        if (d == 0) store_win(&winres[(size_t)w * 4 + 3], tot);
    }
}

static constexpr unsigned DIMBITS_STRIDE = 25;
template <class F>
__global__ __launch_bounds__(64, AccumWaves<F>::W) void k_dimbits(const XYZZ<F> *dims, MsmGeom g, XYZZ<typename WinOut<F>::type> *winres) {
    using LV = LaneView<F>; using E = typename LV::E;
    constexpr unsigned LL = 64 / LV::LANES;
    __shared__ XYZZ<E> sh[64];
    const unsigned n0 = 1u << g.q0, n1 = 1u << g.q1;
    const unsigned per_w = dims_per_w(g);
    const unsigned w = blockIdx.x / DIMBITS_STRIDE, slot = blockIdx.x % DIMBITS_STRIDE;
    const unsigned dtot = g.q2 ? 0u : 1u;
    const unsigned d = slot == 24 ? dtot : slot / g.bd, j = slot % g.bd;
    const unsigned qd = d == 0 ? g.q0 : (d == 1 ? g.q1 : g.q2);
    const bool live = slot == 24 || (d < 3 && j < qd);
    const unsigned doff = d == 0 ? 0 : (d == 1 ? n0 : n0 + n1);
    const unsigned count = !live ? 0u : (slot == 24 ? (1u << qd) : (1u << (qd - 1)));
    const unsigned t = threadIdx.x / LV::LANES;
    XYZZ<E> acc = XYZZ<E>::inf();
    for (unsigned u = t; u < count; u += LL) {
        const unsigned v = slot == 24 ? u : (((u >> j) << (j + 1)) | (1u << j) | (u & ((1u << j) - 1u)));
        xyzz_add(acc, LV::load(&dims[(size_t)w * per_w + doff + v]));
    }
    sh[threadIdx.x] = acc;
    __syncthreads();
    for (unsigned s2 = LL / 2; s2 >= 1; s2 >>= 1) {
        if (t < s2) { xyzz_add(acc, sh[threadIdx.x + s2 * LV::LANES]); sh[threadIdx.x] = acc; }
        __syncthreads();
    }
    if (t == 0) store_win(&winres[(size_t)w * DIMBITS_STRIDE + slot], acc);
}

__device__ __forceinline__ Fp curve_b_mont(const Fp &) { Fp four = Fp::one(); four = dbl(dbl(four)); return four; }
__device__ __forceinline__ Fp2 curve_b_mont(const Fp2 &) { Fp2 b; b.c0 = dbl(dbl(Fp::one())); b.c1 = b.c0; return b; }
template <class F> __global__ __launch_bounds__(256) void k_bases_to_mont(const Affine<F> *in, Affine<F> *out, size_t n, int check_curve, uint32_t *flag) {
    size_t i = (size_t)blockIdx.x * blockDim.x + threadIdx.x;
    if (i >= n) return;
    Affine<F> p = in[i];
    uint32_t bad = (canon_below_p(p.x) && canon_below_p(p.y)) ? 0u : 1u;
    const bool inf = is_zero(p.x) && is_zero(p.y);
    p.x = to_mont(p.x); p.y = to_mont(p.y);
    if (check_curve && !inf && !bad) {
        F rhs = add(mul(sqr(p.x), p.x), curve_b_mont(p.x));
        if (!eq(sqr(p.y), rhs)) bad |= 2u;
    }
    if (bad) atomicOr(flag, bad);
    out[i] = p;
}

static constexpr uint64_t BLS_ABS_Z = 0xd201000000010000ULL;
template <class E> __device__ __noinline__ void sgc_dbl(XYZZ<E> *a) { *a = xyzz_dbl(*a); }
template <class E> __device__ __noinline__ void sgc_madd(XYZZ<E> *a, const Affine<E> *p, bool negate) { XYZZ<E> t = *a; xyzz_madd(t, *p, negate); *a = t; }
template <class E> __device__ __noinline__ void sgc_add(XYZZ<E> *a, const XYZZ<E> *q) { XYZZ<E> t = *a; xyzz_add(t, *q); *a = t; }
template <class F>
__global__ __launch_bounds__(MSM_THREADS, AccumWaves<F>::W) void k_subgroup_check(const Affine<F> *__restrict__ bases, size_t n, uint32_t *flag, uint8_t *status) {
    using LV = LaneView<F>; using E = typename LV::E;
    const size_t i = gid<F>();
    if (i >= n) return;
    Affine<E> p = LV::load(&bases[i]);
    if (is_inf(p)) return;
    XYZZ<E> t1 = xyzz_from_affine(p);
#pragma unroll 1
    for (int b = 62; b >= 0; b--) { sgc_dbl(&t1); if ((BLS_ABS_Z >> b) & 1ull) sgc_madd(&t1, &p, false); }
    XYZZ<E> t2 = t1;
#pragma unroll 1
    for (int b = 62; b >= 0; b--) { sgc_dbl(&t2); if ((BLS_ABS_Z >> b) & 1ull) sgc_add(&t2, &t1); }
    sgc_madd(&t2, &p, true);
    Affine<E> q = p;
    glv_apply(q.x);
    E lx, ly;
    mul_pair(q.x, t2.ZZ, q.y, t2.ZZZ, lx, ly);
    const bool inf2 = is_inf(t2);
    const bool ex = is_zero(sub(lx, t2.X));
    const bool ey = is_zero(sub(ly, t2.Y));
    if (inf2 || !ex || !ey) {
        if (status) status[i] |= 4u;
        else atomicOr(flag, 4u);
    }
}

template <class FT> static bool use_dimbits(long forced, const MsmGeom &g) {
    const size_t cap = g.K > 1 ? ((size_t)64 << 20) : MsmWork::PINNED_BYTES;
    const bool want = forced >= 0 ? forced != 0 : (LaneView<FT>::LANES == 1 || g.Wr <= 2 || g.c > 16);
    return want && (size_t)g.Wr * DIMBITS_STRIDE * sizeof(XYZZ<typename WinOut<FT>::type>) <= cap;
}
template <class FT>
static int launch_tail(vsp_ctx *ctx, hipStream_t st, const MsmWork *pl, const MsmGeom &g, bool dimbits, XYZZ<FT> *buckets, XYZZ<FT> *partials, XYZZ<FT> *dims,
                       XYZZ<typename WinOut<FT>::type> *winres, XYZZ<typename WinOut<FT>::type> *winres_host) {
    using F = FT;
    constexpr unsigned NT = MsmBlock<F>::NT;
    const unsigned per_w = dims_per_w(g);
    {
        const double est = (double)g.n * g.W / (double)g.G / (double)(g.T ? g.T : 1);
        const unsigned lpb = g.single ? 4u : (est < 0.6 ? 16u : (est <= 3.0 ? 1u : 4u));
        const unsigned per_block = MergeBlock<F>::NTL / lpb;
        const size_t want = (g.G + per_block - 1) / per_block;
        const dim3 grid((unsigned)(want < 4096 ? want : 4096));
        const uint32_t *medium = (const uint32_t *)pl->medium.p, *counters = (const uint32_t *)pl->counters.p, *suboff = (const uint32_t *)pl->suboff.p;
        const unsigned sb = lpb == 16 ? (grid.x < 1024 ? grid.x : 1024) : grid.x, all = sb + MERGE1_BLOCKS;
        const uint32_t *heavy = (const uint32_t *)pl->heavy.p;
        if (lpb == 16) hipLaunchKernelGGL(HIP_KERNEL_NAME(k_merge_a<F, 16>), dim3(all), dim3(MergeBlock<F>::NT), 0, st, medium, heavy, counters, suboff, partials, buckets, sb);
        else if (lpb == 4) hipLaunchKernelGGL(HIP_KERNEL_NAME(k_merge_a<F, 4>), dim3(all), dim3(MergeBlock<F>::NT), 0, st, medium, heavy, counters, suboff, partials, buckets, sb);
        else hipLaunchKernelGGL(HIP_KERNEL_NAME(k_merge_a<F, 1>), dim3(all), dim3(MergeBlock<F>::NT), 0, st, medium, heavy, counters, suboff, partials, buckets, sb);
    }
    hipLaunchKernelGGL(HIP_KERNEL_NAME(k_merge2<F>), dim3(256), dim3(MergeBlock<F>::NT), 0, st, (const uint32_t *)pl->heavy.p, (const uint32_t *)pl->counters.p,
                       (const uint32_t *)pl->suboff.p, (const XYZZ<F> *)partials, buckets);
    VSP_LAUNCH_CHECK();
    {
        constexpr unsigned LL = 64 / LaneView<F>::LANES;
        const unsigned sums = g.Wr * per_w;
        unsigned minq = g.q0 < g.q1 ? g.q0 : g.q1; if (g.q2 && g.q2 < minq) minq = g.q2;
        const unsigned items = g.B >> minq;
        unsigned lps = 16; size_t best = ~(size_t)0;
        for (unsigned cand = 8, lg = 3; cand <= LL; cand *= 2, lg++) {
            const size_t waves = ((size_t)sums * cand + LL - 1) / LL;
            const size_t rounds = (waves + DimSumWaves<F>::MAX - 1) / DimSumWaves<F>::MAX;
            const size_t cost = ((items + cand - 1) / cand + lg) * rounds;
            if (cost < best) { best = cost; lps = cand; }
        }
        long forced_lanes = 0;
        { const long t = opt(ctx, "msm_dimsum_lanes", 0); if (t == 8 || t == 16 || t == 32 || (t == 64 && LL == 64)) { lps = (unsigned)t; forced_lanes = t; } }
        const unsigned spw = LL / lps;
        const dim3 grid((sums + spw - 1) / spw);
        DimSumPlan pl; pl.wave0[3] = 0;
        const long mw = opt(ctx, "msm_dimsum_maxw", 1024); const unsigned maxw = mw >= 256 && mw <= 4096 ? (unsigned)mw : 1024u;
        if (!forced_lanes) pl = dimsum_plan<F>(g, maxw);
        ctx->stats["msm_dimsum_waves"] = pl.wave0[3];
        const long pf = opt(ctx, "msm_dimsum_prefetch", 0);
        bool dense = false;
        if constexpr (LaneView<F>::LANES == 1) {
            if (pl.wave0[3] && !pf && opt(ctx, "msm_dimsum_dense", 1)) {
                const unsigned nd[3] = {1u << g.q0, 1u << g.q1, dims_n2(g)};
                DimSumDensePlan dp; dp.blk0[0] = 0;
                for (unsigned d = 0; d < 3; d++) {
                    dp.lps[d] = pl.lps[d];
                    dp.blk0[d + 1] = dp.blk0[d] + (unsigned)(((size_t)g.Wr * nd[d] * pl.lps[d] + DIMSUM_DENSE_NT - 1) / DIMSUM_DENSE_NT);
                }
                hipLaunchKernelGGL(HIP_KERNEL_NAME(k_dimsum_dense<F>), dim3(dp.blk0[3]), dim3(DIMSUM_DENSE_NT), 0, st, (const XYZZ<F> *)buckets, g, dims, dp);
                ctx->stats["msm_dimsum_dense_launches"] += 1;
                dense = true;
            }
        }
        if (dense) {}
        else if (pl.wave0[3] && pf && LaneView<F>::LANES == 1) hipLaunchKernelGGL(HIP_KERNEL_NAME(k_dimsum_mixed<F, true>), dim3(pl.wave0[3]), dim3(64), 0, st, (const XYZZ<F> *)buckets, g, dims, pl);
        else if (pl.wave0[3]) hipLaunchKernelGGL(HIP_KERNEL_NAME(k_dimsum_mixed<F, false>), dim3(pl.wave0[3]), dim3(64), 0, st, (const XYZZ<F> *)buckets, g, dims, pl);
        else
        if (lps == 8) hipLaunchKernelGGL(HIP_KERNEL_NAME(k_dimsum<F, 8>), grid, dim3(64), 0, st, (const XYZZ<F> *)buckets, g, dims);
        else if (lps == 16) hipLaunchKernelGGL(HIP_KERNEL_NAME(k_dimsum<F, 16>), grid, dim3(64), 0, st, (const XYZZ<F> *)buckets, g, dims);
        else if (lps == 32) hipLaunchKernelGGL(HIP_KERNEL_NAME(k_dimsum<F, 32>), grid, dim3(64), 0, st, (const XYZZ<F> *)buckets, g, dims);
        else hipLaunchKernelGGL(HIP_KERNEL_NAME(k_dimsum<F, (LL == 64 ? 64u : 32u)>), grid, dim3(64), 0, st, (const XYZZ<F> *)buckets, g, dims);
    }
    VSP_LAUNCH_CHECK();
    if (dimbits) {
        hipLaunchKernelGGL(HIP_KERNEL_NAME(k_dimbits<F>), dim3(g.Wr * DIMBITS_STRIDE), dim3(64), 0, st, (const XYZZ<F> *)dims, g, winres_host);
    } else {
        hipLaunchKernelGGL(HIP_KERNEL_NAME(k_dimweight<F>), dim3(g.Wr * 3u), dim3(NT), 0, st, (const XYZZ<F> *)dims, g, winres_host);
    }
    VSP_LAUNCH_CHECK();
    return VSP_OK;
}

static unsigned pick_window_bits(vsp_ctx *ctx, long forced, size_t n, bool glv) {
    if (forced >= 2 && forced <= 23) return (unsigned)forced;
    unsigned L = ceil_log2(n ? n : 1);
    int c = (int)L - 4;
    if (c < 4) c = 4;
    if (c > 16) c = 16;
    if (glv && c < 16 && n >= ((size_t)1 << (VSP_MSM_GROUP == 1 ? 18 : 19))) c = 16;
    const long wide = opt(ctx, "msm_wide_windows", 1);
    if (c == 16 && wide && !glv && n >= ((size_t)1 << 20)) c = 17;
    if (c >= 16 && wide && n >= ((size_t)1 << 23)) {
        double best = 0; int bc = 16;
        for (int k = 16; k <= 23; k++) {
            const double W = glv ? (double)((128 + k - 1) / k) : (double)((255 % k == 0 ? 254 : 255) / k + 1);
            const double cost = (double)n * W * (k > 16 ? 0.87 : 1.0) + W * (double)((size_t)1 << (k - 1)) * 4.1;
            if (k == 16 || cost < best) { best = cost; bc = k; }
        }
        c = bc;
    }
    return (unsigned)c;
}

#if VSP_MSM_GROUP == 1
using F28 = Fp28; using Row28 = Affine28;
#else
using F28 = Fp2x28; using Row28 = Affine28x2;
#endif

template <class F> static int msm_geometry(vsp_ctx *ctx, MsmWork &wk, MsmLaunch &L, MsmGeom &g, size_t &n_eff) {
    const MsmPre *pre = L.rq.pre; const bool glv = L.rq.glv; const size_t n = L.rq.n; const unsigned batch = L.rq.batch;
    const uint32_t imul = glv ? 2u : 1u;
    n_eff = n;
    if (L.plan_from) {
        g = L.plan_from->g; n_eff = L.plan_from->n_eff;
        if (L.plan_from->n != n) return set_error(ctx, VSP_ERR_ARG, "msm: shared plan of a different size");
        if ((g.single != 0) != (pre != nullptr) || (pre && (g.idx_stride != pre->stride * imul || g.idx_first != pre->first * imul || g.c != pre->c)))
            return set_error(ctx, VSP_ERR_ARG, "msm: shared plan needs bases precomputed alike");
    } else {
        VSP_TRY(ensure_w(ctx, L.st, wk.counters, 64));
        wk.check_pending = false;
        if (!L.rq.dense) {
            if (!(wk.census_pending && wk.census_n == n && wk.census_scalars == (const void *)L.rq.scalars)) VSP_TRY(msm_census(ctx, wk, L.rq.scalars, n, nullptr, batch, L.rq.stride));
            wk.check_pending = true;
            if (n >= 4096) {
                if (wk.neff_cache_n == n && !opt(ctx, "msm_census_sync", 0)) n_eff = wk.neff_cache;
                else {
                    VSP_HIP(hipEventSynchronize(wk.census_done));
                    uint32_t h_cnt = *(volatile uint32_t *)wk.h_census / batch;
                    n_eff = h_cnt < 256 ? 256 : h_cnt;
                }
            }
        }
        wk.census_pending = false;
        if (glv) n_eff *= 2;
        g.c = pre ? pre->c : pick_window_bits(ctx, L.tune.window_bits, n_eff, glv);
        g.sbits = glv ? 128u : 255u;
        g.fold = (!glv && opt(ctx, "msm_fold", 1) && 255u % g.c == 0u) ? 1u : 0u;
        if (batch > 1 && g.c > 16) g.c = 16;
        if (batch > 1 && g.c < 7) g.c = 7;
        g.Wk = glv ? (128u + g.c - 1) / g.c : (g.fold ? 254u / g.c + 1 : g.sbits / g.c + 1);
        g.K = batch; g.kstride = batch > 1 ? L.rq.stride : 0;
        g.W = g.Wk * g.K;
        g.B = 1u << (g.c - 1);
        g.lb = g.c > 16 ? g.c - 16 : 0u;
        g.n = glv ? 2 * n : n;
        g.single = pre ? 1u : 0u; g.idx_stride = pre ? (uint32_t)(pre->stride * imul) : 0u; g.idx_first = pre ? (uint32_t)(pre->first * imul) : 0u;
        g.Wr = pre ? g.K : g.W;
// ... 120 lines not shown
    L.table28 = rq.pre ? rq.pre->table28 : rq.table28;
    L.rq.glv = rq.glv && (rq.pre ? rq.pre->glv && rq.pre->table28 : rq.table28 != nullptr);
    if (n >= ((size_t)1 << (L.rq.glv ? 30 : 31))) return set_error(ctx, VSP_ERR_UNSUPPORTED, "msm: n >= 2^31");
    L.plan_from = plan_from && plan_from->glv == L.rq.glv ? plan_from : nullptr;
    wk.glv = L.rq.glv;
    L.sort_mode = opt(ctx, "msm_sort", 0);
    L.tune = rq.tuning ? *rq.tuning : MsmTuning{opt(ctx, "msm_window_bits", 0), opt(ctx, "msm_split", 0), opt(ctx, "msm_dimbits", -1)};
    MsmGeom g; size_t n_eff = n;
    VSP_TRY(msm_geometry<F>(ctx, wk, L, g, n_eff));
    wk.g = g; wk.n_eff = n_eff;
    VSP_TRY(msm_split_scalars(ctx, wk, L, g));
    VSP_TRY(msm_buffers<F>(ctx, wk, L, g));
    if (L.plan_from) VSP_HIP(hipStreamWaitEvent(L.st, L.plan_from->plan_ready, 0));
    else { VSP_TRY(msm_digit_sort(ctx, wk, L, g)); VSP_TRY(msm_bucket_plan(ctx, wk, L, g)); }
    if (rq.plan_only) return VSP_OK;
    VSP_TRY(msm_accumulate<F>(ctx, wk, L, g));
    VSP_HIP(hipEventRecord(wk.done, L.st));
    wk.active = true;
    return VSP_OK;
}

template <class F, class HF> static void msm_fold(const MsmWork &wk, XYZZ<HF> *out);
template <class F, class HF>
static int msm_finish_wait(vsp_ctx *ctx, MsmWork &wk, unsigned out_count, bool *empty);
template <class F, class HF>
static int msm_finish(vsp_ctx *ctx, MsmWork &wk, XYZZ<HF> *out, unsigned out_count = 1) {
    for (unsigned k = 0; k < out_count; k++) out[k] = XYZZ<HF>::inf();
    bool empty = false;
    VSP_TRY((msm_finish_wait<F, HF>(ctx, wk, out_count, &empty)));
    if (!empty) msm_fold<F, HF>(wk, out);
    return VSP_OK;
}
template <class F, class HF>
static int msm_finish_wait(vsp_ctx *ctx, MsmWork &wk, unsigned out_count, bool *empty) {
    static_assert(sizeof(F) == sizeof(HF), "host/device field layouts must match");
    *empty = true;
    if (!wk.active) return set_error(ctx, VSP_ERR_ARG, "msm: finish without launch");
    wk.active = false;
    if (wk.empty) return VSP_OK;
    *empty = false;
    if (wk.g.K != out_count) return set_error(ctx, VSP_ERR_ARG, "msm: finish asks for another number of results than the launch's batch");
    VSP_HIP(hipEventSynchronize(wk.done));
    const MsmGeom &g = wk.g;
#ifdef VSP_DEBUG_DUMP
    if (const char *dir = getenv("VSP_DEBUG_DUMP_DIR")) {
        if (FILE *f = fopen((std::string(dir) + "/winres.bin").c_str(), "wb")) { fwrite(wk.h_pinned, 1, (size_t)g.Wr * (wk.dimbits ? DIMBITS_STRIDE : 4) * sizeof(XYZZ<HF>), f); fclose(f); }
        const unsigned per_w = dims_per_w(g);
        std::vector<char> hb(g.G * sizeof(XYZZ<F>)), hd((size_t)g.Wr * per_w * sizeof(XYZZ<F>));
        if (wk.buckets.p && wk.dims.p && hipMemcpy(hb.data(), wk.buckets.p, hb.size(), hipMemcpyDeviceToHost) == hipSuccess &&
            hipMemcpy(hd.data(), wk.dims.p, hd.size(), hipMemcpyDeviceToHost) == hipSuccess) {
            std::string d(dir);
            if (FILE *f = fopen((d + "/buckets.bin").c_str(), "wb")) { fwrite(hb.data(), 1, hb.size(), f); fclose(f); }
            if (FILE *f = fopen((d + "/dims.bin").c_str(), "wb")) { fwrite(hd.data(), 1, hd.size(), f); fclose(f); }
            if (FILE *f = fopen((d + "/geom.txt").c_str(), "w")) { fprintf(f, "%u %u %u %u %u %u %u %zu\n", g.c, g.W, g.Wr, g.B, g.q0, g.q1, g.q2, sizeof(XYZZ<F>)); fclose(f); }
        }
    }
#endif
    if (wk.check_pending) {
        wk.check_pending = false;
        VSP_HIP(hipEventSynchronize(wk.census_done));
        const volatile uint32_t *hc = (const volatile uint32_t *)wk.h_census;
        if (wk.n >= 4096) { const uint32_t c0 = hc[0] / (wk.g.K ? wk.g.K : 1u); wk.neff_cache_n = wk.n; wk.neff_cache = c0 < 256 ? 256 : c0; }
        if (hc[2]) return set_error(ctx, VSP_ERR_ARG, "msm: a scalar is not canonical (>= r)");
    }
    float ms = 0.f;
    if (hipEventElapsedTime(&ms, wk.ev0, wk.ev1) == hipSuccess) {
        ctx->stats["msm_accum_ms"] += ms;
        ctx->stats["msm_accum_launches"] += 1;
    }
    ctx->stats["msm_calls"] += 1;
    ctx->stats["msm_n_eff"] = (double)wk.n_eff;
    ctx->stats["msm_window_bits"] = g.c;
    ctx->stats["msm_windows"] = g.W;
    ctx->stats["msm_bucket_sets"] = g.Wr;
    ctx->stats["msm_split"] = g.T;
    ctx->stats["msm_endomorphism_split"] = wk.glv ? 1 : 0;
    if (opt(ctx, "msm_debug_counts", 0) && wk.counters.p && wk.suboff.p) {
        uint32_t c4[4] = {0, 0, 0, 0}, parts = 0;
        if (hipMemcpy(c4, wk.counters.p, sizeof c4, hipMemcpyDeviceToHost) == hipSuccess &&
            hipMemcpy(&parts, (const uint32_t *)wk.suboff.p + g.G, 4, hipMemcpyDeviceToHost) == hipSuccess) {
            ctx->stats["msm_heavy_buckets"] = c4[0]; ctx->stats["msm_medium_buckets"] = c4[2]; ctx->stats["msm_parts"] = parts;
            ctx->stats["msm_buckets"] = (double)g.G;
        }
    }
    return VSP_OK;
}
template <class F, class HF> static void msm_fold(const MsmWork &wk, XYZZ<HF> *out) {
    const MsmGeom &g = wk.g;
    const XYZZ<HF> *wr = (const XYZZ<HF> *)wk.h_pinned;
    const unsigned per = g.single ? 1u : (g.K > 1 ? g.Wk : g.Wr);
    const bool dimbits_layout = wk.dimbits;
    host_parallel_for(g.K, [&, per, dimbits_layout](size_t kb) {
        XYZZ<HF> acc = XYZZ<HF>::inf();
        const int w_lo = (int)(kb * per), w_hi = (int)(kb * per + per);
        if (dimbits_layout) {
            const unsigned q[3] = {g.q0, g.q1, g.q2};
            for (int w = w_hi - 1; w >= w_lo; w--) {
                const XYZZ<HF> *rec = wr + (size_t)w * DIMBITS_STRIDE;
                acc = xyzz_dbl(acc);
                for (int d = 2; d >= 0; d--)
                    for (int j = (int)q[d] - 1; j >= 0; j--) { acc = xyzz_dbl(acc); xyzz_add(acc, rec[g.bd * d + j]); }
                xyzz_add(acc, rec[24]);
            }
        } else {
            for (int w = w_hi - 1; w >= w_lo; w--) {
                for (unsigned i = 0; i < g.q2 + 1; i++) acc = xyzz_dbl(acc);
                xyzz_add(acc, wr[(size_t)w * 4 + 2]);
                for (unsigned i = 0; i < g.q1; i++) acc = xyzz_dbl(acc);
                xyzz_add(acc, wr[(size_t)w * 4 + 1]);
                for (unsigned i = 0; i < g.q0; i++) acc = xyzz_dbl(acc);
                xyzz_add(acc, wr[(size_t)w * 4 + 0]);
                xyzz_add(acc, wr[(size_t)w * 4 + 3]);
            }
        }
        out[kb] = acc;
    });
}

template <class F> static int launch_slot(vsp_ctx *ctx, unsigned slot_id, const MsmRequest &rq) {
    if (slot_id >= VSP_MSM_SLOTS || rq.plan_from >= (int)VSP_MSM_SLOTS || (rq.batch && rq.plan_from == (int)slot_id)) return set_error(ctx, VSP_ERR_ARG, "msm: bad slot");
    VSP_TRY(work_init(ctx, slot(ctx, slot_id), slot_id == 0 ? ctx->stream : nullptr));
    return msm_launch<F>(ctx, slot(ctx, slot_id), rq, rq.plan_from >= 0 ? &slot(ctx, (unsigned)rq.plan_from) : nullptr);
}

}

template <class G> int msm_precompute(vsp_ctx *ctx, typename G::Point *table, size_t n, unsigned c) {
    using F = typename G::F;
    const unsigned W = 255 / c + 1;
    hipStream_t st = ctx->stream;
    DevBuf tmp, pre;
    VSP_TRY(ensure_w(ctx, st, tmp, n * sizeof(XYZZ<F>)));
    int rc = ensure_w(ctx, st, pre, n * sizeof(F));
    if (rc == VSP_OK) {
        const unsigned blk = (unsigned)((n + MSM_THREADS - 1) / MSM_THREADS);
        const size_t chunks = (n + PRE_CHUNK - 1) / PRE_CHUNK;
        for (unsigned w = 1; w < W; w++) {
            hipLaunchKernelGGL(HIP_KERNEL_NAME(k_shift_window<F>), dim3(blk * LaneView<F>::LANES), dim3(MSM_THREADS), 0, st, (const Affine<F> *)(table + (size_t)(w - 1) * n), n, c, (XYZZ<F> *)tmp.p);
            hipLaunchKernelGGL(HIP_KERNEL_NAME(k_batch_affine_mont<F>), dim3((unsigned)((chunks + 63) / 64)), dim3(64), 0, st, (const XYZZ<F> *)tmp.p, n, (F *)pre.p,
                               table + (size_t)w * n);
        }
        if (hipGetLastError() != hipSuccess || hipStreamSynchronize(st) != hipSuccess) rc = set_error(ctx, VSP_ERR_HIP, "precompute: kernel failed");
    }
    if (tmp.p) hipFree(tmp.p);
    if (pre.p) hipFree(pre.p);
    return rc;
}

template <class G> int msm_table28(vsp_ctx *ctx, const typename G::Point *table, size_t count, void *d_out, bool glv) {
    if (!count) return VSP_OK;
#if defined(VSP_PORTABLE_MUL)
    return VSP_ERR_UNSUPPORTED;
#endif
    hipLaunchKernelGGL(k_table28, dim3((unsigned)((count + 255) / 256)), dim3(256), 0, ctx->stream, table, count, (Row28 *)d_out, glv);
    VSP_LAUNCH_CHECK();
    return VSP_OK;
}
template <class G> int msm_slot_launch(vsp_ctx *ctx, unsigned slot_id, const MsmRequest &rq) { return launch_slot<typename G::F>(ctx, slot_id, rq); }
template <class G> int msm_slot_finish(vsp_ctx *ctx, unsigned slot_id, XYZZ<typename G::HF> *out, unsigned count) {
    return msm_finish<typename G::F, typename G::HF>(ctx, slot(ctx, slot_id), out, count);
}
template <class G> int msm_slot_finish_wait(vsp_ctx *ctx, unsigned slot_id, unsigned count, bool *empty) {
    return msm_finish_wait<typename G::F, typename G::HF>(ctx, slot(ctx, slot_id), count, empty);
}
template <class G> void msm_slot_fold(vsp_ctx *ctx, unsigned slot_id, XYZZ<typename G::HF> *out) { msm_fold<typename G::F, typename G::HF>(slot(ctx, slot_id), out); }
template <class G> int subgroup_check(vsp_ctx *ctx, const typename G::Point *d_mont, size_t n, uint32_t *d_flag, uint8_t *d_status) {
// ... 35 lines not shown
```

Baseline: 369.8 million points/s.

## Route Fp28 reduction-stage point adds through shared noinline XYZZ add/double via LDS pointers

For the 28-bit-limb G1 path, the bucket merge, heavy/medium reductions, dimsum, dimweight and dimbits kernels now call one noinline XYZZ add (plus a wave-uniform fallback double) that reads and writes points through LDS/global pointers. Before, the point arithmetic was inlined at every call site with values kept in registers. The aim is to shrink code size and register pressure, and so raise occupancy in these tail kernels. New call-site variants of the Montgomery asm save the return address in s16/s17 so they can be used inside a noinline function. The cost is more LDS/global traffic and call overhead, plus loops that run to the wave-wide maximum item count. A small early-out for an empty redo list and a debug stat readback are also added.

```diff
diff --git a/vote_saver_protocol_amd/csrc/fp28.h b/vote_saver_protocol_amd/csrc/fp28.h
--- a/vote_saver_protocol_amd/csrc/fp28.h
+++ b/vote_saver_protocol_amd/csrc/fp28.h
@@ -47,6 +47,9 @@
 __device__ __forceinline__ Fp28 mul28(const Fp28 &a, const Fp28 &b) { Fp28 r; mont28_portable(r.l, a.l, b.l, nullptr, nullptr); return r; }
 __device__ __forceinline__ Fp28 sqr28(const Fp28 &a) { Fp28 r; mont28_portable(r.l, a.l, a.l, nullptr, nullptr); return r; }
 __device__ __forceinline__ Fp28 mul28x2(const Fp28 &a, const Fp28 &b, const Fp28 &c, const Fp28 &d) { Fp28 r; mont28_portable(r.l, a.l, b.l, c.l, d.l); return r; }
+__device__ __forceinline__ Fp28 mul28_ra(const Fp28 &a, const Fp28 &b) { return mul28(a, b); }
+__device__ __forceinline__ Fp28 sqr28_ra(const Fp28 &a) { return sqr28(a); }
+__device__ __forceinline__ Fp28 mul28x2_ra(const Fp28 &a, const Fp28 &b, const Fp28 &c, const Fp28 &d) { return mul28x2(a, b, c, d); }
 #else
 __device__ __forceinline__ Fp28 mul28(const Fp28 &a, const Fp28 &b) {
     Fp28 r;
@@ -70,6 +73,32 @@
     Fp28 r;
     __builtin_amdgcn_sched_barrier(0);
     mont_mul28x2_asm(r.l, a.l, b.l, c.l, d.l);
+    __builtin_amdgcn_sched_barrier(0);
+    (void)&mont_mul28x2_holder<0>;
+    return r;
+}
+__device__ __forceinline__ Fp28 mul28_ra(const Fp28 &a, const Fp28 &b) {
+    Fp28 r;
+    __builtin_amdgcn_sched_barrier(0);
+    mont_mul28_asm_ra(r.l, a.l, b.l);
+    __builtin_amdgcn_sched_barrier(0);
+    (void)&mont_mul28_holder<0>;
+    return r;
+}
+__device__ __forceinline__ Fp28 sqr28_ra(const Fp28 &a) {
+    Fp28 r, a2;
+#pragma unroll
+    for (int i = 0; i < 14; i++) a2.l[i] = 2u * a.l[i];
+    __builtin_amdgcn_sched_barrier(0);
+    mont_sqr28_asm_ra(r.l, a.l, a2.l);
+    __builtin_amdgcn_sched_barrier(0);
+    (void)&mont_sqr28_holder<0>;
+    return r;
+}
+__device__ __forceinline__ Fp28 mul28x2_ra(const Fp28 &a, const Fp28 &b, const Fp28 &c, const Fp28 &d) {
+    Fp28 r;
+    __builtin_amdgcn_sched_barrier(0);
+    mont_mul28x2_asm_ra(r.l, a.l, b.l, c.l, d.l);
     __builtin_amdgcn_sched_barrier(0);
     (void)&mont_mul28x2_holder<0>;
     return r;
@@ -228,6 +257,64 @@
     acc.ZZZ = mul28(mul28(acc.ZZZ, q.ZZZ), PPP);
 }
 
+static __device__ __noinline__ __attribute__((not_tail_called)) bool xyzz_add28_shared(XYZZ<Fp28> *dst, const XYZZ<Fp28> *src, bool live) {
+    if (!live) return false;
+    const XYZZ<Fp28> q = *src;
+    if (fp28_all_zero(q.ZZ)) return false;
+    XYZZ<Fp28> acc = *dst;
+    if (fp28_all_zero(acc.ZZ)) { *dst = q; return false; }
+    Fp28 U1 = mul28_ra(acc.X, q.ZZ), U2 = mul28_ra(q.X, acc.ZZ);
+    Fp28 S1 = mul28_ra(acc.Y, q.ZZZ), S2 = mul28_ra(q.Y, acc.ZZZ);
+    Fp28 P = norm28(sub28(U2, FP28_K8_L1, U1));
+    Fp28 PP = sqr28_ra(P);
+    Fp28 R = norm28(sub28(S2, FP28_K8_L1, S1));
+    Fp28 RR = sqr28_ra(R);
+    if (fp28_product_is_zero(PP)) {
+        if (fp28_product_is_zero(RR)) return true;
+        *dst = XYZZ<Fp28>::inf();
+        return false;
+    }
+    Fp28 PPP = mul28_ra(P, PP);
+    Fp28 Q = mul28_ra(U1, PP);
+    Fp28 s;
+#pragma unroll
+    for (int i = 0; i < 14; i++) s.l[i] = PPP.l[i] + 2u * Q.l[i];
+    Fp28 X3 = norm28(sub28(RR, FP28_K8_L4, s));
+    acc.Y = mul28x2_ra(R, sub28(Q, FP28_K32_L1, X3), neg28(FP28_K8_L1, S1), PPP);
+    acc.X = X3;
+    acc.ZZ = mul28_ra(mul28_ra(acc.ZZ, q.ZZ), PP);
+    acc.ZZZ = mul28_ra(mul28_ra(acc.ZZZ, q.ZZZ), PPP);
+    *dst = acc;
+    return false;
+}
+static __device__ __noinline__ __attribute__((not_tail_called)) void xyzz_dbl28_shared(XYZZ<Fp28> *dst, const XYZZ<Fp28> *src, bool live) {
+    if (!live) return;
+    const XYZZ<Fp28> a = *src;
+    XYZZ<Fp28> r;
+    Fp28 U;
+#pragma unroll
+    for (int i = 0; i < 14; i++) U.l[i] = 2u * a.Y.l[i];
+    Fp28 V = mul28_ra(U, U);
+    Fp28 W = mul28_ra(U, V);
+    Fp28 S = mul28_ra(a.X, V);
+    Fp28 M = sqr28_ra(a.X);
+#pragma unroll
+    for (int i = 0; i < 14; i++) M.l[i] *= 3u;
+    M = norm28(M);
+    Fp28 S2;
+#pragma unroll
+    for (int i = 0; i < 14; i++) S2.l[i] = 2u * S.l[i];
+    r.X = norm28(sub28(sqr28_ra(M), FP28_K8_L4, S2));
+    r.Y = mul28x2_ra(M, sub28(S, FP28_K32_L1, r.X), neg28(FP28_K32_L1, a.Y), W);
+    r.ZZ = mul28_ra(V, a.ZZ);
+    r.ZZZ = mul28_ra(W, a.ZZZ);
+    *dst = r;
+}
+__device__ __forceinline__ void tail_add28(XYZZ<Fp28> *dst, const XYZZ<Fp28> *src, bool live) {
+    const bool twice = xyzz_add28_shared(dst, src, live);
+    if (__builtin_amdgcn_ballot_w64(twice) != 0) xyzz_dbl28_shared(dst, src, twice);
+}
+
 
 __device__ __forceinline__ Fp28 partner28(const Fp28 &a) {
     Fp28 r;
@@ -355,6 +442,7 @@
 #else
 __device__ __forceinline__ void xyzz_add(XYZZ<Fp28> &, const XYZZ<Fp28> &) {}
 __device__ __forceinline__ void xyzz_add(XYZZ<Fp28L> &, const XYZZ<Fp28L> &) {}
+__device__ __forceinline__ void tail_add28(XYZZ<Fp28> *, const XYZZ<Fp28> *, bool) {}
 #endif
 
 }
diff --git a/vote_saver_protocol_amd/csrc/mont_asm_gfx950.h b/vote_saver_protocol_amd/csrc/mont_asm_gfx950.h
--- a/vote_saver_protocol_amd/csrc/mont_asm_gfx950.h
+++ b/vote_saver_protocol_amd/csrc/mont_asm_gfx950.h
@@ -1061,6 +1061,7 @@
         "s_branch .Lvsp_mm28_end\n\t"
         ".p2align 8\n\t"
         "vsp_mm28:\n\t"
+        "vsp_mm28_ra:\n\t"
         "s_mov_b32 s0, 0xfffaaab\n\t"
         "s_mov_b32 s1, 0xfefffff\n\t"
         "s_mov_b32 s2, 0x3ffffb9\n\t"
@@ -1556,11 +1557,23 @@
         : "{v0}"(a[0]), "{v1}"(a[1]), "{v2}"(a[2]), "{v3}"(a[3]), "{v4}"(a[4]), "{v5}"(a[5]), "{v6}"(a[6]), "{v7}"(a[7]), "{v8}"(a[8]), "{v9}"(a[9]), "{v10}"(a[10]), "{v11}"(a[11]), "{v12}"(a[12]), "{v13}"(a[13]), "{v14}"(b[0]), "{v15}"(b[1]), "{v16}"(b[2]), "{v17}"(b[3]), "{v18}"(b[4]), "{v19}"(b[5]), "{v20}"(b[6]), "{v21}"(b[7]), "{v22}"(b[8]), "{v23}"(b[9]), "{v24}"(b[10]), "{v25}"(b[11]), "{v26}"(b[12]), "{v27}"(b[13])
         : "vcc", "scc", "s30", "s31", "s0", "s1", "s2", "s3", "s4", "s5", "s6", "s7", "s8", "s9", "s10", "s11", "s12", "s13", "s14", "s15", "v42", "v43", "v44");
 }
+__device__ __forceinline__ void mont_mul28_asm_ra(uint32_t *r, const uint32_t *a, const uint32_t *b) {
+    asm("s_mov_b64 s[16:17], s[30:31]\n\t"
+        "s_getpc_b64 s[30:31]\n\t"
+        "s_add_u32 s30, s30, vsp_mm28_ra@rel32@lo+4\n\t"
+        "s_addc_u32 s31, s31, vsp_mm28_ra@rel32@hi+12\n\t"
+        "s_swappc_b64 s[30:31], s[30:31]\n\t"
+        "s_mov_b64 s[30:31], s[16:17]"
+        : "={v28}"(r[0]), "={v29}"(r[1]), "={v30}"(r[2]), "={v31}"(r[3]), "={v32}"(r[4]), "={v33}"(r[5]), "={v34}"(r[6]), "={v35}"(r[7]), "={v36}"(r[8]), "={v37}"(r[9]), "={v38}"(r[10]), "={v39}"(r[11]), "={v40}"(r[12]), "={v41}"(r[13])
+        : "{v0}"(a[0]), "{v1}"(a[1]), "{v2}"(a[2]), "{v3}"(a[3]), "{v4}"(a[4]), "{v5}"(a[5]), "{v6}"(a[6]), "{v7}"(a[7]), "{v8}"(a[8]), "{v9}"(a[9]), "{v10}"(a[10]), "{v11}"(a[11]), "{v12}"(a[12]), "{v13}"(a[13]), "{v14}"(b[0]), "{v15}"(b[1]), "{v16}"(b[2]), "{v17}"(b[3]), "{v18}"(b[4]), "{v19}"(b[5]), "{v20}"(b[6]), "{v21}"(b[7]), "{v22}"(b[8]), "{v23}"(b[9]), "{v24}"(b[10]), "{v25}"(b[11]), "{v26}"(b[12]), "{v27}"(b[13])
+        : "vcc", "scc", "s16", "s17", "s0", "s1", "s2", "s3", "s4", "s5", "s6", "s7", "s8", "s9", "s10", "s11", "s12", "s13", "s14", "s15", "v42", "v43", "v44");
+}
 template <int Instance> __device__ __attribute__((noinline, used)) void mont_sqr28_holder() {
     asm volatile(
         "s_branch .Lvsp_sq28_end\n\t"
         ".p2align 8\n\t"
         "vsp_sq28:\n\t"
+        "vsp_sq28_ra:\n\t"
         "s_mov_b32 s0, 0xfffaaab\n\t"
         "s_mov_b32 s1, 0xfefffff\n\t"
         "s_mov_b32 s2, 0x3ffffb9\n\t"
@@ -1965,11 +1978,23 @@
         : "{v0}"(a[0]), "{v1}"(a[1]), "{v2}"(a[2]), "{v3}"(a[3]), "{v4}"(a[4]), "{v5}"(a[5]), "{v6}"(a[6]), "{v7}"(a[7]), "{v8}"(a[8]), "{v9}"(a[9]), "{v10}"(a[10]), "{v11}"(a[11]), "{v12}"(a[12]), "{v13}"(a[13]), "{v14}"(a2[0]), "{v15}"(a2[1]), "{v16}"(a2[2]), "{v17}"(a2[3]), "{v18}"(a2[4]), "{v19}"(a2[5]), "{v20}"(a2[6]), "{v21}"(a2[7]), "{v22}"(a2[8]), "{v23}"(a2[9]), "{v24}"(a2[10]), "{v25}"(a2[11]), "{v26}"(a2[12]), "{v27}"(a2[13])
         : "vcc", "scc", "s30", "s31", "s0", "s1", "s2", "s3", "s4", "s5", "s6", "s7", "s8", "s9", "s10", "s11", "s12", "s13", "s14", "s15", "v42", "v43", "v44");
 }
+__device__ __forceinline__ void mont_sqr28_asm_ra(uint32_t *r, const uint32_t *a, const uint32_t *a2) {
+    asm("s_mov_b64 s[16:17], s[30:31]\n\t"
+        "s_getpc_b64 s[30:31]\n\t"
+        "s_add_u32 s30, s30, vsp_sq28_ra@rel32@lo+4\n\t"
+        "s_addc_u32 s31, s31, vsp_sq28_ra@rel32@hi+12\n\t"
+        "s_swappc_b64 s[30:31], s[30:31]\n\t"
+        "s_mov_b64 s[30:31], s[16:17]"
+        : "={v28}"(r[0]), "={v29}"(r[1]), "={v30}"(r[2]), "={v31}"(r[3]), "={v32}"(r[4]), "={v33}"(r[5]), "={v34}"(r[6]), "={v35}"(r[7]), "={v36}"(r[8]), "={v37}"(r[9]), "={v38}"(r[10]), "={v39}"(r[11]), "={v40}"(r[12]), "={v41}"(r[13])
+        : "{v0}"(a[0]), "{v1}"(a[1]), "{v2}"(a[2]), "{v3}"(a[3]), "{v4}"(a[4]), "{v5}"(a[5]), "{v6}"(a[6]), "{v7}"(a[7]), "{v8}"(a[8]), "{v9}"(a[9]), "{v10}"(a[10]), "{v11}"(a[11]), "{v12}"(a[12]), "{v13}"(a[13]), "{v14}"(a2[0]), "{v15}"(a2[1]), "{v16}"(a2[2]), "{v17}"(a2[3]), "{v18}"(a2[4]), "{v19}"(a2[5]), "{v20}"(a2[6]), "{v21}"(a2[7]), "{v22}"(a2[8]), "{v23}"(a2[9]), "{v24}"(a2[10]), "{v25}"(a2[11]), "{v26}"(a2[12]), "{v27}"(a2[13])
+        : "vcc", "scc", "s16", "s17", "s0", "s1", "s2", "s3", "s4", "s5", "s6", "s7", "s8", "s9", "s10", "s11", "s12", "s13", "s14", "s15", "v42", "v43", "v44");
+}
 template <int Instance> __device__ __attribute__((noinline, used)) void mont_mul28x2_holder() {
     asm volatile(
         "s_branch .Lvsp_mm28x2_end\n\t"
         ".p2align 8\n\t"
         "vsp_mm28x2:\n\t"
+        "vsp_mm28x2_ra:\n\t"
         "s_mov_b32 s0, 0xfffaaab\n\t"
         "s_mov_b32 s1, 0xfefffff\n\t"
         "s_mov_b32 s2, 0x3ffffb9\n\t"
@@ -2661,6 +2686,17 @@
         : "{v0}"(a[0]), "{v1}"(a[1]), "{v2}"(a[2]), "{v3}"(a[3]), "{v4}"(a[4]), "{v5}"(a[5]), "{v6}"(a[6]), "{v7}"(a[7]), "{v8}"(a[8]), "{v9}"(a[9]), "{v10}"(a[10]), "{v11}"(a[11]), "{v12}"(a[12]), "{v13}"(a[13]), "{v14}"(b[0]), "{v15}"(b[1]), "{v16}"(b[2]), "{v17}"(b[3]), "{v18}"(b[4]), "{v19}"(b[5]), "{v20}"(b[6]), "{v21}"(b[7]), "{v22}"(b[8]), "{v23}"(b[9]), "{v24}"(b[10]), "{v25}"(b[11]), "{v26}"(b[12]), "{v27}"(b[13]), "{v28}"(c[0]), "{v29}"(c[1]), "{v30}"(c[2]), "{v31}"(c[3]), "{v32}"(c[4]), "{v33}"(c[5]), "{v34}"(c[6]), "{v35}"(c[7]), "{v36}"(c[8]), "{v37}"(c[9]), "{v38}"(c[10]), "{v39}"(c[11]), "{v40}"(c[12]), "{v41}"(c[13]), "{v42}"(d[0]), "{v43}"(d[1]), "{v44}"(d[2]), "{v45}"(d[3]), "{v46}"(d[4]), "{v47}"(d[5]), "{v48}"(d[6]), "{v49}"(d[7]), "{v50}"(d[8]), "{v51}"(d[9]), "{v52}"(d[10]), "{v53}"(d[11]), "{v54}"(d[12]), "{v55}"(d[13])
         : "vcc", "scc", "s30", "s31", "s0", "s1", "s2", "s3", "s4", "s5", "s6", "s7", "s8", "s9", "s10", "s11", "s12", "s13", "s14", "s15", "v70", "v71", "v72");
 }
+__device__ __forceinline__ void mont_mul28x2_asm_ra(uint32_t *r, const uint32_t *a, const uint32_t *b, const uint32_t *c, const uint32_t *d) {
+    asm("s_mov_b64 s[16:17], s[30:31]\n\t"
+        "s_getpc_b64 s[30:31]\n\t"
+        "s_add_u32 s30, s30, vsp_mm28x2_ra@rel32@lo+4\n\t"
+        "s_addc_u32 s31, s31, vsp_mm28x2_ra@rel32@hi+12\n\t"
+        "s_swappc_b64 s[30:31], s[30:31]\n\t"
+        "s_mov_b64 s[30:31], s[16:17]"
+        : "={v56}"(r[0]), "={v57}"(r[1]), "={v58}"(r[2]), "={v59}"(r[3]), "={v60}"(r[4]), "={v61}"(r[5]), "={v62}"(r[6]), "={v63}"(r[7]), "={v64}"(r[8]), "={v65}"(r[9]), "={v66}"(r[10]), "={v67}"(r[11]), "={v68}"(r[12]), "={v69}"(r[13])
+        : "{v0}"(a[0]), "{v1}"(a[1]), "{v2}"(a[2]), "{v3}"(a[3]), "{v4}"(a[4]), "{v5}"(a[5]), "{v6}"(a[6]), "{v7}"(a[7]), "{v8}"(a[8]), "{v9}"(a[9]), "{v10}"(a[10]), "{v11}"(a[11]), "{v12}"(a[12]), "{v13}"(a[13]), "{v14}"(b[0]), "{v15}"(b[1]), "{v16}"(b[2]), "{v17}"(b[3]), "{v18}"(b[4]), "{v19}"(b[5]), "{v20}"(b[6]), "{v21}"(b[7]), "{v22}"(b[8]), "{v23}"(b[9]), "{v24}"(b[10]), "{v25}"(b[11]), "{v26}"(b[12]), "{v27}"(b[13]), "{v28}"(c[0]), "{v29}"(c[1]), "{v30}"(c[2]), "{v31}"(c[3]), "{v32}"(c[4]), "{v33}"(c[5]), "{v34}"(c[6]), "{v35}"(c[7]), "{v36}"(c[8]), "{v37}"(c[9]), "{v38}"(c[10]), "{v39}"(c[11]), "{v40}"(c[12]), "{v41}"(c[13]), "{v42}"(d[0]), "{v43}"(d[1]), "{v44}"(d[2]), "{v45}"(d[3]), "{v46}"(d[4]), "{v47}"(d[5]), "{v48}"(d[6]), "{v49}"(d[7]), "{v50}"(d[8]), "{v51}"(d[9]), "{v52}"(d[10]), "{v53}"(d[11]), "{v54}"(d[12]), "{v55}"(d[13])
+        : "vcc", "scc", "s16", "s17", "s0", "s1", "s2", "s3", "s4", "s5", "s6", "s7", "s8", "s9", "s10", "s11", "s12", "s13", "s14", "s15", "v70", "v71", "v72");
+}
 
 static constexpr uint32_t FR29_R[9] = {0x1u, 0x1ffffff8u, 0x1f96ffbfu, 0x1b4805ffu, 0x1d80553bu, 0xc0404d0u, 0x1520cce7u, 0xa6533afu, 0x73eda7u};
 static constexpr uint32_t FR29_ONE[9] = {0x1fffffbau, 0x22fu, 0x1cb61180u, 0xa4e5c00u, 0xee8b1a2u, 0x16e6aedfu, 0x1907f8bbu, 0x853ddf7u, 0x4d043fu};
diff --git a/vote_saver_protocol_amd/csrc/msm_impl.inc b/vote_saver_protocol_amd/csrc/msm_impl.inc
--- a/vote_saver_protocol_amd/csrc/msm_impl.inc
+++ b/vote_saver_protocol_amd/csrc/msm_impl.inc
@@ -90,6 +90,7 @@
                                                             const uint32_t *__restrict__ part_bucket, XYZZ<F> *buckets, XYZZ<F> *partials,
                                                             const uint32_t *redo_list, const uint32_t *redo_count, bool glv, Bucket28 *b28, Bucket28 *p28) {
     const uint32_t count = *redo_count;
+    if (count == 0) return;
     for (size_t t = gid<F>(); t < count; t += (size_t)gridDim.x * blockDim.x / LaneView<F>::LANES) {
         const uint32_t q = redo_list[t];
         auto acc = accumulate_part<F>(bases, sorted, off, suboff, part_bucket, q, buckets, partials, glv);
@@ -264,6 +265,20 @@
     return acc;
 }
 
+template <class F> struct SharedLaw { static constexpr bool on = false; };
+#if VSP_MSM_GROUP == 1 && !defined(VSP_PORTABLE_MUL)
+template <> struct SharedLaw<Fp28> { static constexpr bool on = true; };
+template <unsigned NT> __device__ __forceinline__ void block_sum28(XYZZ<Fp28> *sh) {
+    const unsigned t = threadIdx.x;
+    for (unsigned s = NT / 2; s >= 1; s >>= 1) {
+        if ((t & ~63u) < s) tail_add28(&sh[t], &sh[t < s ? t + s : t], t < s);
+        __syncthreads();
+    }
+}
+#else
+template <unsigned NT> __device__ __forceinline__ void block_sum28(XYZZ<Fp28> *) {}
+#endif
+
 template <class F> struct MsmBlock { static constexpr unsigned NT = 256; static constexpr unsigned NTL = NT / LaneView<F>::LANES; };
 #ifndef VSP_MERGE_NT
 #define VSP_MERGE_NT 256
@@ -287,9 +302,16 @@
         const uint64_t c0 = (uint64_t)q0 + (uint64_t)k * NTL;
         if (c0 >= q1) continue;
         const uint32_t q = (uint32_t)c0 + lid<F>();
-        XYZZ<E> acc = q < q1 ? LV::load(&partials[q]) : XYZZ<E>::inf();
-        acc = block_sum<F, NT>(acc, sh);
-        if (lid<F>() == 0) LV::store(&partials[c0], acc);
+        if constexpr (SharedLaw<F>::on) {
+            sh[threadIdx.x] = q < q1 ? partials[q] : XYZZ<E>::inf();
+            __syncthreads();
+            block_sum28<NT>(sh);
+            if (threadIdx.x == 0) partials[c0] = sh[0];
+        } else {
+            XYZZ<E> acc = q < q1 ? LV::load(&partials[q]) : XYZZ<E>::inf();
+            acc = block_sum<F, NT>(acc, sh);
+            if (lid<F>() == 0) LV::store(&partials[c0], acc);
+        }
         __syncthreads();
     }
 }
@@ -304,10 +326,21 @@
         uint32_t g = heavy[h];
         uint32_t q0 = suboff[g], q1 = suboff[g + 1];
         const uint32_t stride = (q1 - q0 <= NTL) ? 1u : NTL;
-        XYZZ<E> acc = XYZZ<E>::inf();
-        for (uint32_t q = q0 + lid<F>() * stride; q < q1; q += NTL * stride) xyzz_add(acc, LV::load(&partials[q]));
-        acc = block_sum<F, NT>(acc, sh);
-        if (lid<F>() == 0) LV::store(&buckets[g], acc);
+        if constexpr (SharedLaw<F>::on) {
+            sh[threadIdx.x] = XYZZ<E>::inf();
+            for (uint64_t qb = q0; qb < q1; qb += (uint64_t)NTL * stride) {
+                const uint64_t q = qb + (uint64_t)threadIdx.x * stride;
+                tail_add28(&sh[threadIdx.x], &partials[q < q1 ? q : q0], q < q1);
+            }
+            __syncthreads();
+            block_sum28<NT>(sh);
+            if (threadIdx.x == 0) buckets[g] = sh[0];
+        } else {
+            XYZZ<E> acc = XYZZ<E>::inf();
+            for (uint32_t q = q0 + lid<F>() * stride; q < q1; q += NTL * stride) xyzz_add(acc, LV::load(&partials[q]));
+            acc = block_sum<F, NT>(acc, sh);
+            if (lid<F>() == 0) LV::store(&buckets[g], acc);
+        }
         __syncthreads();
     }
 }
@@ -330,17 +363,31 @@
         const bool live = t < nm;
         const uint32_t g = live ? medium[t] : 0u;
         const uint32_t q0 = live ? suboff[g] : 0u, q1 = live ? suboff[g + 1] : 0u;
-        XYZZ<E> acc = XYZZ<E>::inf();
-        for (uint32_t q = q0 + lane; q < q1; q += LPB) xyzz_add(acc, LV::load(&partials[q]));
-        if constexpr (LPB > 1) {
-            sh[threadIdx.x] = acc;
-            __syncthreads();
-            for (unsigned s = LPB / 2; s >= 1; s >>= 1) {
-                if (lane < s) { xyzz_add(acc, sh[threadIdx.x + s * LV::LANES]); sh[threadIdx.x] = acc; }
+        if constexpr (SharedLaw<F>::on) {
+            XYZZ<E> *mine = &sh[threadIdx.x];
+            *mine = XYZZ<E>::inf();
+            for (uint32_t q = q0 + lane; __builtin_amdgcn_ballot_w64(q < q1) != 0; q += LPB) tail_add28(mine, &partials[q < q1 ? q : q0], q < q1);
+            if constexpr (LPB > 1) {
                 __syncthreads();
+                for (unsigned s = LPB / 2; s >= 1; s >>= 1) {
+                    tail_add28(mine, lane < s ? mine + s : mine, lane < s);
+                    __syncthreads();
+                }
             }
-        }
-        if (live && lane == 0) LV::store(&buckets[g], acc);
+            if (live && lane == 0) buckets[g] = *mine;
+        } else {
+            XYZZ<E> acc = XYZZ<E>::inf();
+            for (uint32_t q = q0 + lane; q < q1; q += LPB) xyzz_add(acc, LV::load(&partials[q]));
+            if constexpr (LPB > 1) {
+                sh[threadIdx.x] = acc;
+                __syncthreads();
+                for (unsigned s = LPB / 2; s >= 1; s >>= 1) {
+                    if (lane < s) { xyzz_add(acc, sh[threadIdx.x + s * LV::LANES]); sh[threadIdx.x] = acc; }
+                    __syncthreads();
+                }
+            }
+            if (live && lane == 0) LV::store(&buckets[g], acc);
+        }
     }
 }
 
@@ -413,6 +460,24 @@
     const unsigned qd = d == 0 ? g.q0 : (d == 1 ? g.q1 : g.q2);
     const unsigned items = live ? g.B >> qd : 0;
     const XYZZ<F> *bw = buckets + (size_t)w * g.B;
+    if constexpr (SharedLaw<F>::on) {
+        XYZZ<E> *mine = &sh[threadIdx.x];
+        *mine = XYZZ<E>::inf();
+        for (unsigned i = lane; __builtin_amdgcn_ballot_w64(i < items) != 0; i += LPS) {
+            unsigned idx;
+            if (d == 0) idx = (i << g.q0) | v;
+            else if (d == 1) idx = ((i >> g.q0) << (g.q1 + g.q0)) | (v << g.q0) | (i & (n0 - 1));
+            else idx = (v << (g.q1 + g.q0)) | i;
+            tail_add28(mine, &bw[i < items ? idx : 0u], i < items);
+        }
+        __syncthreads();
+        for (unsigned s = LPS / 2; s >= 1; s >>= 1) {
+            tail_add28(mine, lane < s ? mine + s : mine, lane < s);
+            __syncthreads();
+        }
+        if (live && lane == 0) dims[(size_t)w * per_w + slot] = *mine;
+        return;
+    }
     XYZZ<E> acc = XYZZ<E>::inf();
     for (unsigned i = lane; i < items; i += LPS) {
         unsigned idx;
@@ -454,6 +519,19 @@
         if (d == 1) return ((i >> g.q0) << (g.q1 + g.q0)) | (v << g.q0) | (i & (n0 - 1));
         return (v << (g.q1 + g.q0)) | i;
     };
+    if constexpr (SharedLaw<F>::on) {
+        XYZZ<E> *mine = &sh[threadIdx.x];
+        *mine = XYZZ<E>::inf();
+        const unsigned all_items = g.B >> qd;
+        for (unsigned i = lane; i - lane < all_items; i += LPS) tail_add28(mine, &bw[i < items ? index_of(i) : 0u], i < items);
+        __syncthreads();
+        for (unsigned s = LPS / 2; s >= 1; s >>= 1) {
+            tail_add28(mine, lane < s ? mine + s : mine, lane < s);
+            __syncthreads();
+        }
+        if (live && lane == 0) dims[(size_t)w * per_w + base + v] = *mine;
+        return;
+    }
     XYZZ<E> acc = XYZZ<E>::inf();
     if constexpr (LANES == 1 && PREFETCH) {
         XYZZ<E> nxt = lane < items ? LV::load(&bw[index_of(lane)]) : XYZZ<E>::inf();
@@ -500,14 +578,32 @@
             if (d == 1) return ((i >> g.q0) << (g.q1 + g.q0)) | (v << g.q0) | (i & (n0 - 1));
             return (v << (g.q1 + g.q0)) | i;
         };
-        XYZZ<E> acc = XYZZ<E>::inf();
-        for (unsigned i = lane; i < items; i += LPS) xyzz_add(acc, LV::load(&bw[index_of(i)]));
-        sh[threadIdx.x] = acc;
+        if constexpr (SharedLaw<F>::on) {
+            XYZZ<E> *mine = &sh[threadIdx.x];
+            *mine = XYZZ<E>::inf();
+            const unsigned all_items = g.B >> qd;
+            for (unsigned i = lane; i - lane < all_items; i += LPS) tail_add28(mine, &bw[i < items ? index_of(i) : 0u], i < items);
+        } else {
+            XYZZ<E> acc = XYZZ<E>::inf();
+            for (unsigned i = lane; i < items; i += LPS) xyzz_add(acc, LV::load(&bw[index_of(i)]));
+            sh[threadIdx.x] = acc;
+        }
     }
     __syncthreads();
     const unsigned wave_first = threadIdx.x & ~63u;
     for (unsigned s = LPS / 2; s >= 1; s >>= 1) {
         const unsigned A = SPB * s;
+        if constexpr (SharedLaw<F>::on) {
+            if (wave_first < A) {
+                const unsigned j = threadIdx.x;
+                const unsigned slot = j < A ? (j / s) * LPS + j % s : 0u;
+                tail_add28(&sh[slot], &sh[slot + s], j < A);
+                if (s == 1 && j < A) {
+                    const unsigned id = id0 + j;
+                    if (id < g.Wr * nd) dims[(size_t)(id / nd) * per_w + base + id % nd] = sh[slot];
+                }
+            }
+        } else
         if (wave_first < A) {
             const unsigned j = threadIdx.x;
             if (j < A) {
@@ -563,6 +659,19 @@
     *p = xyzz28_to_fp(v);
 #endif
 }
+__device__ __forceinline__ void store_win28(XYZZ<Fp> *p, const XYZZ<Fp28> *v) {
+#if defined(__HIP_DEVICE_COMPILE__)
+    const Fp28 *in = &v->X;
+    Fp *out = &p->X;
+    const bool inf = fp28_all_zero(v->ZZ);
+#pragma unroll 1
+    for (int k = 0; k < 4; k++) {
+        Fp r = Fp::zero();
+        if (!inf) r = fp28_to_fp(in[k]);
+        out[k] = r;
+    }
+#endif
+}
 __device__ __forceinline__ void store_win(XYZZ<Fp2> *p, const XYZZ<Fp28L> &v) {
 #if defined(__HIP_DEVICE_COMPILE__)
     Fp *row = reinterpret_cast<Fp *>(p);
@@ -587,6 +696,27 @@
     const unsigned cntv = d == 0 ? n0 : (d == 1 ? n1 : n2);
     const unsigned doff = d == 0 ? 0 : (d == 1 ? n0 : n0 + n1);
     const unsigned t = lid<F>();
+    if constexpr (SharedLaw<F>::on) {
+        XYZZ<E> *gd = const_cast<XYZZ<E> *>(&dims[(size_t)w * per_w + doff]);
+        XYZZ<E> *cur = gd, *nxt = sh;
+        for (unsigned s = 1; s < cntv; s <<= 1) {
+            const bool mine = t < cntv, add = mine && t + s < cntv;
+            if (mine) nxt[t] = cur[t];
+            tail_add28(&nxt[t < cntv ? t : 0], &cur[add ? t + s : 0], add);
+            __syncthreads();
+            XYZZ<E> *sw = cur; cur = nxt; nxt = sw;
+        }
+        if (t == 0 && cur != gd) gd[0] = cur[0];
+        __syncthreads();
+        sh[t] = (t >= 1 && t < cntv) ? cur[t] : XYZZ<E>::inf();
+        __syncthreads();
+        block_sum28<NT>(sh);
+        if (t == 0) {
+#pragma unroll 1
+            for (unsigned k = 0; k < (d == 0 ? 2u : 1u); k++) store_win28(&winres[(size_t)w * 4 + (k ? 3u : d)], k ? &gd[0] : &sh[0]);
+        }
+        return;
+    }
     XYZZ<E> x = t < cntv ? LV::load(&dims[(size_t)w * per_w + doff + t]) : XYZZ<E>::inf();
     sh[at<F>(t)] = x;
     __syncthreads();
@@ -623,6 +753,21 @@
     const unsigned doff = d == 0 ? 0 : (d == 1 ? n0 : n0 + n1);
     const unsigned count = !live ? 0u : (slot == 24 ? (1u << qd) : (1u << (qd - 1)));
     const unsigned t = threadIdx.x / LV::LANES;
+    if constexpr (SharedLaw<F>::on) {
+        XYZZ<E> *mine = &sh[threadIdx.x];
+        *mine = XYZZ<E>::inf();
+        for (unsigned u = t; u - t < count; u += LL) {
+            const unsigned v = slot == 24 ? u : (((u >> j) << (j + 1)) | (1u << j) | (u & ((1u << j) - 1u)));
+            tail_add28(mine, &dims[(size_t)w * per_w + doff + (u < count ? v : 0u)], u < count);
+        }
+        __syncthreads();
+        for (unsigned s2 = LL / 2; s2 >= 1; s2 >>= 1) {
+            tail_add28(mine, t < s2 ? mine + s2 : mine, t < s2);
+            __syncthreads();
+        }
+        if (t == 0) store_win28(&winres[(size_t)w * DIMBITS_STRIDE + slot], &sh[0]);
+        return;
+    }
     XYZZ<E> acc = XYZZ<E>::inf();
     for (unsigned u = t; u < count; u += LL) {
         const unsigned v = slot == 24 ? u : (((u >> j) << (j + 1)) | (1u << j) | (u & ((1u << j) - 1u)));
@@ -747,8 +892,9 @@
                 dense = true;
             }
         }
+        constexpr bool has_prefetch = LaneView<F>::LANES == 1 && !SharedLaw<F>::on;
         if (dense) {}
-        else if (pl.wave0[3] && pf && LaneView<F>::LANES == 1) hipLaunchKernelGGL(HIP_KERNEL_NAME(k_dimsum_mixed<F, true>), dim3(pl.wave0[3]), dim3(64), 0, st, (const XYZZ<F> *)buckets, g, dims, pl);
+        else if (pl.wave0[3] && pf && has_prefetch) hipLaunchKernelGGL(HIP_KERNEL_NAME(k_dimsum_mixed<F, has_prefetch>), dim3(pl.wave0[3]), dim3(64), 0, st, (const XYZZ<F> *)buckets, g, dims, pl);
         else if (pl.wave0[3]) hipLaunchKernelGGL(HIP_KERNEL_NAME(k_dimsum_mixed<F, false>), dim3(pl.wave0[3]), dim3(64), 0, st, (const XYZZ<F> *)buckets, g, dims, pl);
         else
         if (lps == 8) hipLaunchKernelGGL(HIP_KERNEL_NAME(k_dimsum<F, 8>), grid, dim3(64), 0, st, (const XYZZ<F> *)buckets, g, dims);
@@ -1035,6 +1181,8 @@
             ctx->stats["msm_heavy_buckets"] = c4[0]; ctx->stats["msm_medium_buckets"] = c4[2]; ctx->stats["msm_parts"] = parts;
             ctx->stats["msm_buckets"] = (double)g.G;
         }
+        uint32_t redone = 0;
+        if (wk.redo.p && hipMemcpy(&redone, wk.redo.p, 4, hipMemcpyDeviceToHost) == hipSuccess) ctx->stats["msm_redo_parts"] = redone;
     }
     return VSP_OK;
 }
```

Measured after the change: 370.3 million points/s (median of 2 runs). Within noise of the previous version (+0.1%).
